# xhchrn/D-LADMM

Hardware: AMD Instinct MI355X
Metric: samples/sec through d=15 D-LADMM forward (m=256,n=512); %HBM-roofline (higher is better)
Workload: dtype f32; 1 GPU; DLADMMNet_scalar (V4) forward m=256 n=512 K=15 B=65536/GPU, all layers' Z/E/L/T written + fused per-layer L1L1 objective; variant=v4, m=256, n=512, layers=15, batch_per_gpu=65536, global_batch=65536, keep_all=True, parallelism=batch-shard dp1 (one RCCL all-reduce of [K,2] sums)

## Files before the change

### d-ladmm_amd/_lib.py

```python
from __future__ import annotations

import ctypes
import os

HERE = os.path.dirname(os.path.abspath(__file__))
LIB_PATH = os.environ.get("DLADMM_LIB") or os.path.join(HERE, "lib", "libdladmm_hip.so")

ABI_VERSION = 6
PREC_F32, PREC_BF16, PREC_F32_SPLIT = 0, 1, 2
MAX_LAYERS = 65536
NSCALAR = 8

F_PER_LAYER, F_BF16_WIDE, F_BWD_PER_LAYER, F_BWD_UNFUSED, F_BWD_NO_ZMASK, F_WGRAD_F32 = \
    1, 2, 4, 8, 16, 32
F_NO_ROWSPLIT = 64
F_NO_XSPLIT = 128
F_ROWSPLIT_ROWP = 256
F_P0_SAVE = 512
F_P0_REUSE = 1024
F_ELZ = 2048
F_ELZ_TAIL = 4096
V1_LENA, V2_LTHETA, V3_FULL, V4_SCALAR, V5_TIED, V6_LASSO = 1, 2, 3, 4, 5, 6
V7_SCALAR_V1E = 7
LOSS_NONE, LOSS_L1L1, LOSS_LASSO = 0, 1, 2
P_BETA1, P_BETA2, P_BETA3, P_SS2, P_SS2B, P_THETA_E, P_THETA_Z, P_S1 = range(8)

EXPORTED = ("dladmm_abi_version", "dladmm_fwd_workspace_bytes", "dladmm_fwd_path",
            "dladmm_fwd_f32", "dladmm_bwd_workspace_bytes", "dladmm_bwd_path", "dladmm_bwd_f32",
            "dladmm_safeguard_f32", "dladmm_safeguard_news_f32", "dladmm_colobj_f32", "dladmm_lena_workspace_bytes",
            "dladmm_lena_f32", "dladmm_scale_f32", "dladmm_error_string")
MU_NONE, MU_EMA, MU_GS, MU_RT = 0, 1, 2, 3

_fp = ctypes.c_void_p
_i32 = ctypes.c_int32
_i64 = ctypes.c_int64


class FwdDesc(ctypes.Structure):
    _fields_ = [
        ("abi_version", _i32), ("variant", _i32), ("m", _i32), ("n", _i32),
        ("batch", _i32), ("layers", _i32), ("keep_all", _i32), ("loss_kind", _i32),
        ("X", _fp), ("ld_x", _i64),
        ("A", _fp), ("ld_a", _i64),
        ("Z0", _fp), ("ld_z0", _i64),
        ("E0", _fp), ("ld_e0", _i64),
        ("L0", _fp), ("ld_l0", _i64),
        ("W", ctypes.POINTER(_fp)), ("ld_w", _i64),
        ("scalar_params", _fp),
        ("row_params", _fp), ("row_stride", _i64),
        ("beta1_elem", ctypes.POINTER(_fp)),
        ("beta2_elem", ctypes.POINTER(_fp)),
        ("ld_beta", _i64),
        ("Z", _fp), ("E", _fp), ("L", _fp), ("T", _fp),
        ("ld_out", _i64),
        ("loss_sums", _fp),
        ("workspace", _fp), ("workspace_bytes", ctypes.c_size_t),
        ("ev_kernel_start", _fp), ("ev_kernel_stop", _fp),
        ("col_loss", _fp),
        ("precision", _i32), ("flags", _i32),
        ("P", _fp),
    ]


class BwdDesc(ctypes.Structure):
    _fields_ = [
        ("fwd", FwdDesc),
        ("gZ", ctypes.POINTER(_fp)), ("gE", ctypes.POINTER(_fp)), ("gL", ctypes.POINTER(_fp)),
        ("gT", ctypes.POINTER(_fp)), ("ld_g", _i64),
        ("loss_kind", _i32), ("gw_sum", _i32), ("loss_coef", _fp),
        ("gW", _fp), ("ld_gw", _i64),
        ("g_scalar", _fp), ("g_row", _fp),
        ("g_beta1_elem", ctypes.POINTER(_fp)), ("g_beta2_elem", ctypes.POINTER(_fp)),
        ("workspace", _fp), ("workspace_bytes", ctypes.c_size_t),
    ]


class SafeguardDesc(ctypes.Structure):
    _fields_ = [
        ("abi_version", _i32), ("m", _i32), ("n", _i32), ("batch", _i32), ("ld", _i64),
        ("Zl", _fp), ("El", _fp), ("Ll", _fp), ("Tl", _fp),
        ("Zk", _fp), ("Ek", _fp), ("Lk", _fp), ("Tk", _fp),
        ("Es", _fp), ("Ts", _fp), ("Ep", _fp),
        ("Zo", _fp), ("Eo", _fp), ("Lo", _fp), ("To", _fp),
        ("mu", _fp), ("norm_out", _fp), ("count", _fp),
        ("beta", ctypes.c_float), ("c", ctypes.c_float), ("delta", ctypes.c_double),
        ("updater", _i32), ("mu_param", ctypes.c_float),
    ]


class SafeguardNewsDesc(ctypes.Structure):
    _fields_ = [
        ("abi_version", _i32), ("m", _i32), ("n", _i32), ("batch", _i32), ("ld", _i64),
        ("X", _fp),
        ("Zl", _fp), ("El", _fp), ("Ll", _fp),
        ("Zk", _fp), ("Ek", _fp), ("Lk", _fp),
        ("En", _fp), ("Znn", _fp), ("Pn", _fp), ("Pnn", _fp),
        ("Zo", _fp), ("Eo", _fp), ("Lo", _fp),
        ("mu", _fp), ("norm_out", _fp), ("count", _fp), ("mask", _fp), ("inv_bs", _fp),
        ("delta", ctypes.c_double), ("updater", _i32), ("mu_param", ctypes.c_float),
    ]


class ColObjDesc(ctypes.Structure):
    _fields_ = [
        ("abi_version", _i32), ("m", _i32), ("n", _i32), ("batch", _i32), ("layers", _i32),
        ("fit_kind", _i32),
        ("Z", _fp), ("z_layer_stride", _i64), ("ld_z", _i64),
        ("E", _fp), ("e_layer_stride", _i64), ("ld_e", _i64),
        ("T", _fp), ("t_layer_stride", _i64), ("ld_t", _i64),
        ("Zref", _fp), ("ld_zref", _i64),
        ("Eref", _fp), ("ld_eref", _i64),
        ("reg", _fp), ("fit", _fp), ("dz", _fp), ("de", _fp),
    ]


class LenaDesc(ctypes.Structure):
    _fields_ = [
        ("abi_version", _i32), ("m", _i32), ("n", _i32), ("batch", _i32), ("layers", _i32),
        ("mode", _i32), ("alpha", ctypes.c_float), ("inv_mb", ctypes.c_float),
        ("inv_nb", ctypes.c_float), ("lx_negate", _i32),
        ("X", _fp), ("ld_x", _i64), ("A", _fp), ("ld_a", _i64),
        ("E", _fp), ("L", _fp), ("layer_stride", _i64), ("ld", _i64),
        ("sums", _fp),
        ("gE", _fp), ("gL", _fp), ("g_layer_stride", _i64), ("ld_g", _i64),
        ("coef", _fp),
        ("workspace", _fp), ("workspace_bytes", ctypes.c_size_t),
    ]


_LIB = None


def lib():
    global _LIB
    if _LIB is not None:
        return _LIB
    if not os.path.exists(LIB_PATH):
        raise RuntimeError(
            f"dladmm: HIP library not built ({LIB_PATH} missing); run "
            "`python -c 'import __graft_entry__ as g; g.build()'` or `make -C d-ladmm_amd`")
    import torch
    L = ctypes.CDLL(LIB_PATH)
    L.dladmm_abi_version.restype = ctypes.c_int
    L.dladmm_abi_version.argtypes = []
    L.dladmm_fwd_workspace_bytes.restype = ctypes.c_size_t
    L.dladmm_fwd_workspace_bytes.argtypes = [ctypes.POINTER(FwdDesc)]
    L.dladmm_fwd_path.restype = ctypes.c_int
    L.dladmm_fwd_path.argtypes = [ctypes.POINTER(FwdDesc)]
    L.dladmm_fwd_f32.restype = ctypes.c_int
    L.dladmm_fwd_f32.argtypes = [ctypes.POINTER(FwdDesc), ctypes.c_void_p]
    L.dladmm_bwd_workspace_bytes.restype = ctypes.c_size_t
    L.dladmm_bwd_workspace_bytes.argtypes = [ctypes.POINTER(BwdDesc)]
    L.dladmm_bwd_path.restype = ctypes.c_int
    L.dladmm_bwd_path.argtypes = [ctypes.POINTER(BwdDesc)]
    L.dladmm_bwd_f32.restype = ctypes.c_int
    L.dladmm_bwd_f32.argtypes = [ctypes.POINTER(BwdDesc), ctypes.c_void_p]
    L.dladmm_safeguard_f32.restype = ctypes.c_int
    L.dladmm_safeguard_f32.argtypes = [ctypes.POINTER(SafeguardDesc), ctypes.c_void_p]
    L.dladmm_safeguard_news_f32.restype = ctypes.c_int
    L.dladmm_safeguard_news_f32.argtypes = [ctypes.POINTER(SafeguardNewsDesc), ctypes.c_void_p]
    L.dladmm_colobj_f32.restype = ctypes.c_int
    L.dladmm_colobj_f32.argtypes = [ctypes.POINTER(ColObjDesc), ctypes.c_void_p]
    L.dladmm_lena_workspace_bytes.restype = ctypes.c_size_t
    L.dladmm_lena_workspace_bytes.argtypes = [ctypes.POINTER(LenaDesc)]
    L.dladmm_lena_f32.restype = ctypes.c_int
    L.dladmm_lena_f32.argtypes = [ctypes.POINTER(LenaDesc), ctypes.c_void_p]
    L.dladmm_scale_f32.restype = ctypes.c_int
    L.dladmm_scale_f32.argtypes = [ctypes.c_void_p, ctypes.c_int64, ctypes.c_void_p, ctypes.c_void_p]
    L.dladmm_error_string.restype = ctypes.c_char_p
    L.dladmm_error_string.argtypes = [ctypes.c_int]
    if L.dladmm_abi_version() != ABI_VERSION:
        raise RuntimeError("dladmm: library ABI version mismatch; rebuild")
    _LIB = L
    return L


def check(code: int):
    if code != 0:
        msg = lib().dladmm_error_string(code).decode()
        if code < 0:
            raise ValueError(f"{msg} (code {code})")
        raise RuntimeError(f"dladmm HIP error: {msg} (code {code})")


def ptr_array(ptrs):
    arr = (_fp * max(len(ptrs), 1))()
    for i, p in enumerate(ptrs):
        arr[i] = p
    return arr
```

### d-ladmm_amd/csrc/dladmm_capi.hip

```cpp
#include <math.h>
#include <stdlib.h>

#include <vector>

#include "dladmm_common.h"
#include "dladmm_wgrad_x3.h"
#include "dladmm_internal.h"

namespace dladmm {

constexpr int kPackBatch = 64;

struct PackArgs {
  const float* src[kPackBatch];
  int R, C, RB, CB;
  int order;
  int64_t ld;
  float* dst;
  float sign;
  const float* scal;
  int trans;
  int t0;
  int bf16;
  int vec;
};
static_assert(sizeof(PackArgs) <= 2048, "kernel argument size");

__global__ __launch_bounds__(256) void pack_frags_kernel(const PackArgs p) {
  const int t = blockIdx.y;
  const int64_t fr = (int64_t)blockIdx.x * 4 + (threadIdx.x >> 6);
  if (fr >= (int64_t)p.RB * p.CB) return;
  const int lane = threadIdx.x & 63;
  int ib, jb;
  if (p.order == 0) { ib = (int)(fr / p.CB); jb = (int)(fr % p.CB); }
  else if (p.order == 1) { ib = (int)(fr % p.RB); jb = (int)(fr / p.RB); }
  else { const int64_t q = fr >> 1; jb = (int)(q % p.CB); ib = 2 * (int)(q / p.CB) + (int)(fr & 1); }
  const float f = p.sign * (p.scal ? p.scal[(p.t0 + t) * DLADMM_NSCALAR + DLADMM_P_S1] : 1.0f);
  const int row = 16 * ib + (lane & 15);
  if (p.bf16) {
    const int c8 = 32 * jb + 8 * (lane >> 4);
    const float* s8 = p.src[t];
    bf16x8 v;
    if (p.vec && !p.trans && row < p.R && c8 + 8 <= p.C) {
      const f32x4* q4 = reinterpret_cast<const f32x4*>(s8 + (int64_t)row * p.ld + c8);
      const f32x4 lo = q4[0], hi = q4[1];
#pragma unroll
      for (int q = 0; q < 4; ++q) {
        v[q] = (__bf16)(f * lo[q]);
        v[4 + q] = (__bf16)(f * hi[q]);
      }
      reinterpret_cast<bf16x8*>(p.dst)[((int64_t)t * p.RB * p.CB + fr) * 64 + lane] = v;
      return;
    }
#pragma unroll
    for (int q = 0; q < 8; ++q) {
      const float x = (row < p.R && c8 + q < p.C)
                          ? f * (p.trans ? s8[(int64_t)(c8 + q) * p.ld + row]
                                         : s8[(int64_t)row * p.ld + c8 + q])
                          : 0.0f;
      v[q] = (__bf16)x;
    }
    reinterpret_cast<bf16x8*>(p.dst)[((int64_t)t * p.RB * p.CB + fr) * 64 + lane] = v;
    return;
  }
  const int c0 = 16 * jb + 4 * (lane >> 4);
  const float* s = p.src[t];
  f32x4 v;
  if (p.vec && !p.trans && row < p.R && c0 + 4 <= p.C) {
    const f32x4 x = *reinterpret_cast<const f32x4*>(s + (int64_t)row * p.ld + c0);
#pragma unroll
    for (int q = 0; q < 4; ++q) v[q] = f * x[q];
    reinterpret_cast<f32x4*>(p.dst)[((int64_t)t * p.RB * p.CB + fr) * 64 + lane] = v;
    return;
  }
#pragma unroll
  for (int q = 0; q < 4; ++q)
    v[q] = (row < p.R && c0 + q < p.C)
               ? f * (p.trans ? s[(int64_t)(c0 + q) * p.ld + row] : s[(int64_t)row * p.ld + c0 + q])
               : 0.0f;
  reinterpret_cast<f32x4*>(p.dst)[((int64_t)t * p.RB * p.CB + fr) * 64 + lane] = v;
}

__global__ __launch_bounds__(256) void zero_fill_kernel(uint32_t* p, int64_t words,
                                                        uint8_t* tail, int ntail) {
  const int64_t i0 = (int64_t)blockIdx.x * 256 + threadIdx.x;
  for (int64_t i = i0; i < words; i += (int64_t)gridDim.x * 256) p[i] = 0u;
  if (i0 < ntail) tail[i0] = 0;
}
inline hipError_t zero_async(void* p, size_t bytes, hipStream_t s) {
  if (bytes == 0) return hipSuccess;
  const uintptr_t a = (uintptr_t)p;
  const size_t head = (4 - (a & 3)) & 3;
  if (head) {
    hipLaunchKernelGGL(zero_fill_kernel, dim3(1), dim3(256), 0, s, (uint32_t*)nullptr,
                       (int64_t)0, (uint8_t*)p, (int)(head < bytes ? head : bytes));
    if (hipError_t e = hipGetLastError()) return e;
    if (head >= bytes) return hipSuccess;
    p = (uint8_t*)p + head;
    bytes -= head;
  }
  const int64_t words = (int64_t)(bytes / 4);
  const int ntail = (int)(bytes & 3);
  int64_t blocks = (words + 255) / 256;
  blocks = blocks < 1 ? 1 : (blocks > 1024 ? 1024 : blocks);
  hipLaunchKernelGGL(zero_fill_kernel, dim3((unsigned)blocks), dim3(256), 0, s, (uint32_t*)p,
                     words, (uint8_t*)p + 4 * words, ntail);
  return hipGetLastError();
}

__global__ __launch_bounds__(256) void zero_2d_kernel(float* p, int64_t ld, int cols, int rows) {
  const int64_t t = (int64_t)blockIdx.x * 256 + threadIdx.x;
  if (t < (int64_t)rows * cols) p[(t / cols) * ld + t % cols] = 0.0f;
}
inline hipError_t zero_2d_async(float* p, int64_t ld, int cols, int rows, hipStream_t s) {
  const int64_t total = (int64_t)rows * cols;
  if (total == 0) return hipSuccess;
  hipLaunchKernelGGL(zero_2d_kernel, dim3((unsigned)((total + 255) / 256)), dim3(256), 0, s, p, ld,
                     cols, rows);
  return hipGetLastError();
}

constexpr int kPtrChunk = 64;
struct PtrChunk {
  const void* p[kPtrChunk];
  const void** dst;
  int n;
};
__global__ __launch_bounds__(64) void ptr_table_kernel(const PtrChunk c) {
  if ((int)threadIdx.x < c.n) c.dst[threadIdx.x] = c.p[threadIdx.x];
}
inline hipError_t write_ptr_table(const void* const* src, int n, const void** dst, hipStream_t s) {
  for (int b = 0; b < n; b += kPtrChunk) {
    PtrChunk c{};
    c.n = n - b < kPtrChunk ? n - b : kPtrChunk;
    for (int i = 0; i < c.n; ++i) c.p[i] = src[b + i];
    c.dst = dst + b;
    hipLaunchKernelGGL(ptr_table_kernel, dim3(1), dim3(64), 0, s, c);
    if (hipError_t e = hipGetLastError()) return e;
  }
  return hipSuccess;
}

typedef _Float16 f16x8_t __attribute__((ext_vector_type(8)));
struct X3PackArgs {
  const float* src[kPackBatch];
  int R, C, RB, KS, t0;
  int64_t ld;
  float sign;
  f16x8_t* dst;
  unsigned* umax;
  int* wexp;
};
static_assert(sizeof(X3PackArgs) <= 2048, "kernel argument size");

__global__ __launch_bounds__(256) void absmax_kernel(const X3PackArgs p) {
  const int t = blockIdx.y;
  const float* src = p.src[t];
  const int64_t total = (int64_t)p.R * p.C;
  float mx = 0.0f;
  for (int64_t i = (int64_t)blockIdx.x * 256 + threadIdx.x; i < total; i += (int64_t)gridDim.x * 256)
    mx = fmaxf(mx, fabsf(src[(i / p.C) * p.ld + i % p.C]));
#pragma unroll
  for (int o = 32; o > 0; o >>= 1) mx = fmaxf(mx, __shfl_xor(mx, o, 64));
  __shared__ float red[4];
  if ((threadIdx.x & 63) == 0) red[threadIdx.x >> 6] = mx;
  __syncthreads();
  if (threadIdx.x == 0) {
    mx = fmaxf(fmaxf(red[0], red[1]), fmaxf(red[2], red[3]));
    atomicMax(p.umax + p.t0 + t, __float_as_uint(mx));
  }
}

__global__ __launch_bounds__(256) void pack_x3_kernel(const X3PackArgs p) {
  const int t = blockIdx.y;
  const int st = blockIdx.x * 4 + (threadIdx.x >> 6);
  if (st >= p.RB * p.KS) return;
  const int lane = threadIdx.x & 63;
  const int ib = st / p.KS, ks = st % p.KS;
  int sw = 15 - __builtin_amdgcn_frexp_expf(__uint_as_float(p.umax[p.t0 + t]));
  sw = sw < -126 ? -126 : (sw > 126 ? 126 : sw);
  if (st == 0 && lane == 0) p.wexp[p.t0 + t] = sw;
  const float f = p.sign * __builtin_amdgcn_ldexpf(1.0f, sw);
  const float* src = p.src[t];
  const int row = 16 * ib + (lane & 15);
  f16x8_t hi, lo;
#pragma unroll
  for (int q = 0; q < 8; ++q) {
    const int c = 32 * ks + 16 * (q >> 2) + 4 * (lane >> 4) + (q & 3);
    const float x = (row < p.R && c < p.C) ? src[(int64_t)row * p.ld + c] * f : 0.0f;
    const _Float16 h = (_Float16)x;
    hi[q] = h;
    lo[q] = (_Float16)(x - (float)h);
  }
  f16x8_t* d = p.dst + ((int64_t)t * p.RB * p.KS + st) * 128;
  d[lane] = hi;
  d[64 + lane] = lo;
}

__global__ __launch_bounds__(256) void col_loss_kernel(const float* part, int nslice, int ldl,
                                                       int B, float* out) {
  const int r = blockIdx.y;
  const int b = blockIdx.x * 256 + threadIdx.x;
  if (b >= B) return;
  float s = 0.0f;
  for (int sl = 0; sl < nslice; ++sl) s += part[((int64_t)r * nslice + sl) * ldl + b];
  out[(int64_t)r * B + b] = s;
}

__global__ __launch_bounds__(1024) void param_reduce_kernel(const float* part, int stride,
                                                            int cnt_m, int cnt_n, double* sums) {
  __shared__ double red[1024];
  const int sl = blockIdx.x;
  if (sl == DLADMM_P_S1) {
    if (threadIdx.x == 0) sums[sl] = 0.0;
    return;
  }
  const int cnt = (sl == DLADMM_P_THETA_Z || sl == DLADMM_P_S1) ? cnt_n : cnt_m;
  double s = 0.0;
  for (int w = threadIdx.x; w < cnt; w += 1024) s += (double)part[(int64_t)sl * stride + w];
  red[threadIdx.x] = s;
  __syncthreads();
  for (int o = 512; o > 0; o >>= 1) {
    if ((int)threadIdx.x < o) red[threadIdx.x] += red[threadIdx.x + o];
    __syncthreads();
  }
  if (threadIdx.x == 0) sums[sl] = red[0];
}

__device__ __forceinline__ double fixed_sum_1024(const float* row, int nw, double* red) {
  double acc8[8] = {0, 0, 0, 0, 0, 0, 0, 0};
  int wv = threadIdx.x;
  for (; wv + 7 * 1024 < nw; wv += 8 * 1024) {
#pragma unroll
    for (int u = 0; u < 8; ++u) acc8[u] += (double)row[wv + u * 1024];
  }
  for (int u = 0; wv < nw; wv += 1024, ++u) acc8[u & 7] += (double)row[wv];
  double s = 0.0;
#pragma unroll
  for (int u = 0; u < 8; ++u) s += acc8[u];
  red[threadIdx.x] = s;
  __syncthreads();
  for (int o = 512; o > 0; o >>= 1) {
    if ((int)threadIdx.x < o) red[threadIdx.x] += red[threadIdx.x + o];
    __syncthreads();
  }
  return red[0];
}

__global__ __launch_bounds__(1024) void loss_reduce_kernel(const float* part, int nw, double* sums) {
  __shared__ double red[1024];
  const int i = blockIdx.x;
  const double s = fixed_sum_1024(part + (int64_t)i * nw, nw, red);
  if (threadIdx.x == 0) sums[i] = s;
}

__global__ __launch_bounds__(1024) void row_reduce_kernel(const float* part, int nw, int prs,
                                                          int ors, int m, int n, unsigned mask,
                                                          double* out) {
  __shared__ double red[1024];
  const int i = blockIdx.x;
  const int row = i % ors, ks = i / ors;
  const int slot = ks % 8;
  const bool ok = ((mask >> slot) & 1u) && row < (slot == DLADMM_P_THETA_Z ? n : m);
  if (!ok) {
    if (threadIdx.x == 0) out[i] = 0.0;
    return;
  }
  const double s = fixed_sum_1024(part + ((int64_t)ks * prs + row) * nw, nw, red);
  if (threadIdx.x == 0) out[i] = s;
}

}

namespace dladmm {

inline size_t align256(size_t x) { return (x + 255) & ~(size_t)255; }

inline int pick_shape(int m, int n) {
  for (int i = 0; i < kNumShapes; ++i)
    if (m <= kShapeMP[i] && n <= kShapeNP[i]) return i;
  return -1;
}

inline int ceil_div(int a, int b) { return (a + b - 1) / b; }

struct Plan {
  int path;
  int shape, MP, NP, tiles;
  int KB1, KB2, SB1, SB2, MBp1, MBp2, slices1, slices2, gx;
  int nslots;
  int ldl;
  int nbp;
  bool narrow;
  size_t off_ap, off_wp, off_v, off_zb, off_zw, off_ew, off_lw, off_loss, total;
  size_t off_btab;
  size_t off_xch, off_xcnt;
  size_t off_wexp, off_umax;
  bool p0;
  size_t off_p0;
  int64_t ldzw;
};

inline bool fits_32bit(const dladmm_fwd_desc* d);

inline int validate(const dladmm_fwd_desc* d) {
  if (!d) return DLADMM_E_NULL;
  if (d->abi_version != DLADMM_ABI_VERSION) return DLADMM_E_ABI_VERSION;
  if (d->variant < DLADMM_V1_LENA || d->variant > DLADMM_V7_SCALAR_V1E) return DLADMM_E_VARIANT;
  if (d->m < 1 || d->n < 1 || d->batch < 1) return DLADMM_E_SHAPE;
  if (d->layers < 1 || d->layers > DLADMM_MAX_LAYERS) return DLADMM_E_LAYERS;
  if (d->loss_kind < 0 || d->loss_kind > 2) return DLADMM_E_UNSUPPORTED;
  if (!d->X || !d->A || !d->Z0 || !d->E0 || !d->L0 || !d->W || !d->Z || !d->E || !d->L)
    return DLADMM_E_NULL;
  for (int k = 0; k < d->layers; ++k)
    if (!d->W[k]) return DLADMM_E_NULL;
  if (d->loss_kind && !d->loss_sums) return DLADMM_E_NULL;
  if (d->col_loss && !d->loss_kind) return DLADMM_E_UNSUPPORTED;
  if (d->precision != DLADMM_PREC_F32 && d->precision != DLADMM_PREC_BF16 &&
      d->precision != DLADMM_PREC_F32_SPLIT)
    return DLADMM_E_UNSUPPORTED;
  const int v = d->variant;
  if (v == DLADMM_V2_LTHETA || v == DLADMM_V3_FULL) {
    if (!d->row_params) return DLADMM_E_NULL;
    if (d->row_stride < d->m || d->row_stride < d->n) return DLADMM_E_SHAPE;
  } else if (!d->scalar_params) {
    return DLADMM_E_NULL;
  }
  if (v == DLADMM_V1_LENA) {
    if (!d->beta1_elem || !d->beta2_elem) return DLADMM_E_NULL;
    for (int k = 0; k < d->layers; ++k)
      if (!d->beta1_elem[k] || !d->beta2_elem[k]) return DLADMM_E_NULL;
    if (d->ld_beta < d->batch) return DLADMM_E_SHAPE;
  }
  const int64_t B = d->batch;
  if (d->ld_x < B || d->ld_z0 < B || d->ld_e0 < B || d->ld_l0 < B || d->ld_out < B)
    return DLADMM_E_SHAPE;
  if (d->ld_a < d->n || d->ld_w < d->m) return DLADMM_E_SHAPE;
  const bool elz = (d->flags & DLADMM_F_ELZ) != 0;
  if (v == DLADMM_V7_SCALAR_V1E || elz) {
    if (d->precision != DLADMM_PREC_F32 || (d->flags & DLADMM_F_PER_LAYER) ||
        pick_shape(d->m, d->n) < 0 || !fits_32bit(d))
      return DLADMM_E_UNSUPPORTED;
    if (v == DLADMM_V7_SCALAR_V1E && d->P && !elz) return DLADMM_E_UNSUPPORTED;
  }
  if (elz) {
    if (v != DLADMM_V4_SCALAR && v != DLADMM_V5_TIED && v != DLADMM_V7_SCALAR_V1E)
      return DLADMM_E_UNSUPPORTED;
    if (!d->keep_all || d->loss_kind) return DLADMM_E_UNSUPPORTED;
  }
  if ((d->flags & DLADMM_F_ELZ_TAIL) && (!elz || !d->P)) return DLADMM_E_UNSUPPORTED;
  return 0;
}

inline bool fits_32bit(const dladmm_fwd_desc* d) {
  const int64_t lim = (int64_t)1 << 31;
  const int64_t mx = d->m > d->n ? d->m : d->n;
  return !(mx * d->ld_x * 4 >= lim || mx * d->ld_z0 * 4 >= lim || mx * d->ld_e0 * 4 >= lim ||
           mx * d->ld_l0 * 4 >= lim || mx * d->ld_out * 4 >= lim ||
           (d->variant == DLADMM_V1_LENA && mx * d->ld_beta * 4 >= lim));
}

inline bool x3_layout_ok(const dladmm_fwd_desc* d) {
  auto al = [](const void* p) { return ((uintptr_t)p & 15) == 0; };
  return d->batch % 4 == 0 && d->ld_out % 4 == 0 && d->ld_z0 % 4 == 0 && al(d->Z0) &&
         al(d->Z) && al(d->E) && al(d->L) && (!d->T || al(d->T));
}

inline bool shared_weight(const dladmm_fwd_desc* d) {
  for (int k = 1; k < d->layers; ++k)
    if (d->W[k] != d->W[0]) return false;
  return true;
}

inline bool use_wgrad_x3(bool x3w, const WgradArgs& wa) { return x3w && wgrad_x3_fits(wa); }

inline int device_cus() {
  static const int n = [] {
    int dev = 0, v = 0;
    if (hipGetDevice(&dev) != hipSuccess ||
        hipDeviceGetAttribute(&v, hipDeviceAttributeMultiprocessorCount, dev) != hipSuccess)
      return 256;
    return v > 0 ? v : 256;
  }();
  return n;
}

#ifndef DLADMM_RS_PER_CU
#define DLADMM_RS_PER_CU 3
#endif
inline bool use_rowsplit(const dladmm_fwd_desc* d, int shape) {
  const bool rowv = d->variant == DLADMM_V2_LTHETA || d->variant == DLADMM_V3_FULL;
  return rs_supports(shape, d->variant) && (!rowv || (d->flags & DLADMM_F_ROWSPLIT_ROWP)) &&
         d->precision == DLADMM_PREC_F32 &&
         !(d->flags & DLADMM_F_NO_ROWSPLIT) &&
         ceil_div(d->batch, 16) <= DLADMM_RS_PER_CU * device_cus();
}

inline bool use_xsplit(const dladmm_fwd_desc* d, int shape) {
  return use_rowsplit(d, shape) && !(d->flags & (DLADMM_F_NO_XSPLIT | DLADMM_F_ELZ)) &&
         xs_grid(d->batch) <= device_cus();
}

inline int make_plan(const dladmm_fwd_desc* d, Plan* p) {
  *p = Plan{};
  const int s = pick_shape(d->m, d->n);
  const int K = d->layers;
  const int64_t B = d->batch;
  const bool force_layered = (d->flags & DLADMM_F_PER_LAYER) != 0;
  const bool bf16 = d->precision == DLADMM_PREC_BF16;
  if (s >= 0 && fits_32bit(d) && !force_layered && d->precision == DLADMM_PREC_F32_SPLIT &&
      x3_supports(d->variant) && x3_layout_ok(d)) {
    p->path = 4;
    p->shape = s < 1 ? 1 : s;
    p->MP = kShapeMP[p->shape];
    p->NP = kShapeNP[p->shape];
    p->tiles = ceil_div(d->batch, kTileCols);
    p->ldl = p->tiles * kTileCols;
    p->nslots = p->ldl;
    p->ldzw = p->ldl;
    const size_t tb = (size_t)p->MP * p->NP * 2 * sizeof(_Float16);
    const int nw = shared_weight(d) ? 1 : K;
    p->off_ap = 0;
    p->off_wp = align256(tb);
    p->off_wexp = p->off_wp + align256(tb * nw);
    p->off_umax = p->off_wexp + align256((size_t)(nw + 1) * sizeof(int));
    p->off_zw = p->off_umax + align256((size_t)(nw + 1) * sizeof(unsigned));
    const bool lean = !d->keep_all && K > 1;
    p->off_loss = p->off_zw + (lean ? align256((size_t)2 * d->n * p->ldzw * sizeof(float)) : 0);
    p->off_btab = p->off_loss + align256((size_t)2 * K * p->nslots * sizeof(float));
    p->total = p->off_btab +
               (d->variant == DLADMM_V1_LENA ? align256((size_t)2 * K * sizeof(void*)) : 0);
    return 0;
  }
  if (s >= 0 && fits_32bit(d) && !force_layered && !bf16) {
    p->path = use_xsplit(d, s) ? 6 : use_rowsplit(d, s) ? 5 : 1;
    p->shape = s;
    p->MP = kShapeMP[s];
    p->NP = kShapeNP[s];
    p->tiles = ceil_div(d->batch, kTileCols);
    p->ldl = p->path >= 5 ? ceil_div(d->batch, 16) * 16 : p->tiles * kTileCols;
    p->nslots = p->ldl;
    const size_t frag_bytes = (size_t)p->MP * p->NP * sizeof(float);
    p->off_ap = 0;
    p->off_wp = align256(frag_bytes);
    p->off_loss = p->off_wp + align256(frag_bytes * (shared_weight(d) ? 1 : K));
    p->off_btab = p->off_loss + align256((size_t)2 * K * p->nslots * sizeof(float));
    p->total = p->off_btab +
               (d->variant == DLADMM_V1_LENA ? align256((size_t)2 * K * sizeof(void*)) : 0);
    if (p->path == 1 && (d->flags & (DLADMM_F_P0_SAVE | DLADMM_F_P0_REUSE)) &&
        !(d->flags & DLADMM_F_ELZ) &&
        d->precision == DLADMM_PREC_F32 && p0_supports(s, d->variant) &&
        (int64_t)p->MP * p->ldl * 4 < ((int64_t)1 << 31)) {
      p->p0 = true;
      p->off_p0 = p->total;
      p->total += align256((size_t)p->MP * p->ldl * sizeof(float));
    }
    if (p->path == 6) {
      const size_t groups = (size_t)xs_grid(d->batch) / 4;
      p->off_xch = p->total;
      p->off_xcnt = p->off_xch + align256(groups * xs_group_floats() * sizeof(float));
      p->total = p->off_xcnt + align256(groups * 64 * sizeof(unsigned));
    }
    return 0;
  }
  p->path = bf16 ? 3 : 2;
  const int MB = ceil_div(d->m, 16), NB = ceil_div(d->n, 16);
  p->KB1 = bf16 ? ceil_div(d->m, 32) : MB;
  p->KB2 = bf16 ? ceil_div(d->n, 32) : NB;
  p->SB1 = bf16 ? kTileBlocks : (NB >= 32 ? 32 : 16);
  p->SB2 = bf16 ? kTileBlocks : (MB >= 32 ? 32 : 16);
  p->MBp1 = ceil_div(NB, p->SB1) * p->SB1;
  p->MBp2 = ceil_div(MB, p->SB2) * p->SB2;
  p->slices1 = p->MBp1 / p->SB1;
  p->slices2 = p->MBp2 / p->SB2;
  p->narrow = bf16 && !(d->flags & DLADMM_F_BF16_WIDE);
  const int cols = bf16 ? bf16_tile_cols(p->narrow) : kLayerCols;
  p->gx = ceil_div(d->batch, cols);
  p->ldl = p->gx * cols;
  p->nbp = p->ldl / 16;
  p->nslots = p->ldl * (p->slices1 > p->slices2 ? p->slices1 : p->slices2) * (bf16 ? 2 : 1);
  const size_t fb = (size_t)kFrag * sizeof(float);
  p->off_ap = 0;
  p->off_wp = align256(fb * p->KB2 * p->MBp2);
  p->off_v = p->off_wp + align256(fb * p->KB1 * p->MBp1 * (shared_weight(d) ? 1 : K));
  p->off_zb = p->off_v + align256(bf16 ? fb * p->KB1 * p->nbp : (size_t)d->m * B * sizeof(float));
  p->off_zw = p->off_zb + (bf16 ? align256(fb * p->KB2 * p->nbp) : 0);
  const bool lean = !d->keep_all && K > 1;
  p->off_ew = p->off_zw + (lean ? align256((size_t)d->n * B * sizeof(float)) : 0);
  p->off_lw = p->off_ew + (lean ? align256((size_t)d->m * B * sizeof(float)) : 0);
  p->off_loss = p->off_lw + (lean ? align256((size_t)d->m * B * sizeof(float)) : 0);
  p->total = p->off_loss + align256((size_t)2 * K * p->nslots * sizeof(float));
  return 0;
}

inline hipError_t pack(const float* const* srcs, int T, int R, int C, int64_t ld, int RB, int CB,
                       int order, float* dst, hipStream_t s, float sign = 1.0f,
                       const float* scal = nullptr, int trans = 0, int t0 = 0, int bf16 = 0) {
  for (int b = 0; b < T; b += kPackBatch) {
    const int nb = T - b < kPackBatch ? T - b : kPackBatch;
    PackArgs pa{};
    pa.trans = trans; pa.t0 = t0 + b;
    for (int t = 0; t < nb; ++t) pa.src[t] = srcs[b + t];
    pa.R = R; pa.C = C; pa.RB = RB; pa.CB = CB; pa.order = order; pa.ld = ld;
    pa.dst = dst + (size_t)b * RB * CB * kFrag;
    pa.sign = sign; pa.scal = scal; pa.bf16 = bf16;
    pa.vec = ld % 4 == 0 ? 1 : 0;
    for (int t = 0; t < nb; ++t)
      if ((uintptr_t)pa.src[t] & 15) pa.vec = 0;
    hipLaunchKernelGGL(pack_frags_kernel, dim3((RB * CB + 3) / 4, nb), dim3(256), 0, s, pa);
    if (hipError_t e = hipGetLastError()) return e;
  }
  return hipSuccess;
}

inline unsigned long long* dbg_ptr() {
#if defined(X3_STAMP) && X3_STAMP
  static unsigned long long* const p = [] {
    const char* e = getenv("DLADMM_DBG_PTR");
    return e ? (unsigned long long*)strtoull(e, nullptr, 0) : nullptr;
  }();
  return p;
#else
  return nullptr;
#endif
}

inline int run_fused(const dladmm_fwd_desc* d, const Plan& p, char* ws, hipStream_t s) {
  float* Ap = (float*)(ws + p.off_ap);
  float* Wp = (float*)(ws + p.off_wp);
  float* lossp = (float*)(ws + p.off_loss);
  const int MB = p.MP / 16, NB = p.NP / 16;
  const float* asrc[1] = {d->A};
  const bool shared = shared_weight(d);
  const bool p0_reuse = p.p0 && !(d->flags & DLADMM_F_P0_SAVE);
  if (!p0_reuse)
    if (hipError_t e = pack(asrc, 1, d->m, d->n, d->ld_a, MB, NB, 2, Ap, s)) return (int)e;
  if (hipError_t e = pack(d->W, shared ? 1 : d->layers, d->n, d->m, d->ld_w, NB, MB, 2, Wp, s,
                          -1.0f))
    return (int)e;
  FusedArgs a{};
  a.m = d->m; a.n = d->n; a.B = d->batch; a.K = d->layers;
  a.keep_all = d->keep_all ? 1 : 0; a.loss_kind = d->loss_kind; a.ldl = p.ldl;
  a.elz = (d->flags & DLADMM_F_ELZ) ? ((d->flags & DLADMM_F_ELZ_TAIL) ? 2 : 1) : 0;
  a.X = d->X; a.ldx = d->ld_x;
  a.Z0 = d->Z0; a.ldz0 = d->ld_z0;
  a.E0 = d->E0; a.lde0 = d->ld_e0;
  a.L0 = d->L0; a.ldl0 = d->ld_l0;
  a.Ap = Ap; a.Wp = Wp;
  a.wstep = shared ? 0 : 1;
  a.scal = d->scalar_params;
  a.rowp = d->row_params; a.rstride = d->row_stride;
  a.ldb = d->ld_beta;
  if (d->variant == DLADMM_V1_LENA) {
    const void** tab = (const void**)(ws + p.off_btab);
    if (hipError_t e = write_ptr_table((const void* const*)d->beta1_elem, d->layers, tab, s))
      return (int)e;
    if (hipError_t e = write_ptr_table((const void* const*)d->beta2_elem, d->layers,
                                       tab + d->layers, s))
      return (int)e;
    a.b1t = (const float* const*)tab;
    a.b2t = (const float* const*)(tab + d->layers);
  }
  a.Zo = d->Z; a.Eo = d->E; a.Lo = d->L; a.To = d->T; a.ldo = d->ld_out;
  a.lossp = lossp;
  a.dbg = dbg_ptr();
  const bool savep = d->P != nullptr && d->keep_all;
  a.Po = savep ? d->P : nullptr;
  if (p.p0) {
    a.P0 = (const float*)(ws + p.off_p0);
    a.ldp0 = p.ldl;
    if (!p0_reuse)
      if (hipError_t e = launch_p0_producer(p.shape, Ap, d->Z0, d->ld_z0, d->n, d->batch,
                                            (float*)(ws + p.off_p0), p.ldl, p.tiles, s))
        return (int)e;
  }
  if (d->ev_kernel_start) {
    if (hipError_t e = hipEventRecord((hipEvent_t)d->ev_kernel_start, s)) return (int)e;
  }
  if (p.path == 6) {
    a.xch = (float*)(ws + p.off_xch);
    a.xstride = (int64_t)xs_group_floats();
    a.xcnt = (unsigned*)(ws + p.off_xcnt);
    if (hipError_t e = zero_async(a.xcnt, p.total - p.off_xcnt, s)) return (int)e;
  }
  hipError_t e = p.path == 6 ? launch_fused_xs(p.shape, d->variant, a, s)
                 : p.path == 5
                    ? launch_fused_rs(p.shape, d->variant, a, ceil_div(d->batch, 16), s)
                 : a.elz ? launch_fused_shape_elz(p.shape, d->variant, a, p.tiles, s)
                 : p0_reuse
                    ? (savep ? launch_fused_shape_p0_savep : launch_fused_shape_p0)(
                          p.shape, d->variant, a, p.tiles, s)
                    : (savep ? launch_fused_shape_savep : launch_fused_shape)(p.shape, d->variant,
                                                                             a, p.tiles, s);
  if (e) return (int)e;
  if (d->ev_kernel_stop) {
    if (hipError_t e = hipEventRecord((hipEvent_t)d->ev_kernel_stop, s)) return (int)e;
  }
  return 0;
}

inline hipError_t pack_x3(const float* const* srcs, int T, int R, int C, int64_t ld, int RB,
                          int KS, float sign, _Float16* dst, unsigned* umax, int* wexp, int t0,
                          hipStream_t s) {
  for (int b = 0; b < T; b += kPackBatch) {
    const int nb = T - b < kPackBatch ? T - b : kPackBatch;
    X3PackArgs pa{};
    for (int t = 0; t < nb; ++t) pa.src[t] = srcs[b + t];
    pa.R = R; pa.C = C; pa.RB = RB; pa.KS = KS; pa.t0 = t0 + b; pa.ld = ld; pa.sign = sign;
    pa.dst = reinterpret_cast<f16x8_t*>(dst) + (size_t)b * RB * KS * 128;
    pa.umax = umax; pa.wexp = wexp;
    const int blocks = ceil_div((int)(((int64_t)R * C + 255) / 256), 8);
    hipLaunchKernelGGL(absmax_kernel, dim3(blocks < 64 ? blocks : 64, nb), dim3(256), 0, s, pa);
    if (hipError_t e = hipGetLastError()) return e;
    hipLaunchKernelGGL(pack_x3_kernel, dim3(ceil_div(RB * KS, 4), nb), dim3(256), 0, s, pa);
    if (hipError_t e = hipGetLastError()) return e;
  }
  return hipSuccess;
}

inline int run_fused_x3(const dladmm_fwd_desc* d, const Plan& p, char* ws, hipStream_t s) {
  _Float16* Ap = (_Float16*)(ws + p.off_ap);
  _Float16* Wp = (_Float16*)(ws + p.off_wp);
  int* wexp = (int*)(ws + p.off_wexp);
  unsigned* umax = (unsigned*)(ws + p.off_umax);
  const int MB = p.MP / 16, NB = p.NP / 16, KS1 = p.MP / 32, KS2 = p.NP / 32;
  const bool shared = shared_weight(d);
  const int nw = shared ? 1 : d->layers;
  if (hipError_t e = zero_async(umax, (size_t)(nw + 1) * sizeof(unsigned), s)) return (int)e;
  const float* asrc[1] = {d->A};
  if (hipError_t e = pack_x3(asrc, 1, d->m, d->n, d->ld_a, MB, KS2, 1.0f, Ap, umax, wexp, 0, s))
    return (int)e;
  if (hipError_t e = pack_x3(d->W, nw, d->n, d->m, d->ld_w, NB, KS1, -1.0f, Wp, umax, wexp, 1, s))
    return (int)e;
  FusedArgs a{};
  a.m = d->m; a.n = d->n; a.B = d->batch; a.K = d->layers;
  a.keep_all = d->keep_all ? 1 : 0; a.loss_kind = d->loss_kind; a.ldl = p.ldl;
  a.X = d->X; a.ldx = d->ld_x;
  a.Z0 = d->Z0; a.ldz0 = d->ld_z0;
  a.E0 = d->E0; a.lde0 = d->ld_e0;
  a.L0 = d->L0; a.ldl0 = d->ld_l0;
  a.Ap = (const float*)Ap; a.Wp = (const float*)Wp;
  a.wstep = shared ? 0 : 1;
  a.scal = d->scalar_params;
  a.Zo = d->Z; a.Eo = d->E; a.Lo = d->L; a.To = d->T; a.ldo = d->ld_out;
  a.lossp = (float*)(ws + p.off_loss);
  a.wexp = wexp;
  a.Zw = (float*)(ws + p.off_zw); a.ldzw = p.ldzw;
  a.dbg = dbg_ptr();
  if (d->variant == DLADMM_V1_LENA) {
    a.ldb = d->ld_beta;
    const void** tab = (const void**)(ws + p.off_btab);
    if (hipError_t e = write_ptr_table((const void* const*)d->beta1_elem, d->layers, tab, s))
      return (int)e;
    if (hipError_t e = write_ptr_table((const void* const*)d->beta2_elem, d->layers,
                                       tab + d->layers, s))
      return (int)e;
    a.b1t = (const float* const*)tab;
    a.b2t = (const float* const*)(tab + d->layers);
  }
  if (d->ev_kernel_start) {
    if (hipError_t e = hipEventRecord((hipEvent_t)d->ev_kernel_start, s)) return (int)e;
  }
  const bool savep = d->P != nullptr && d->keep_all;
  a.Po = savep ? d->P : nullptr;
  if (hipError_t e = (savep ? launch_fused_x3_shape_savep : launch_fused_x3_shape)(
          p.shape, d->variant, a, p.tiles, s))
    return (int)e;
  if (d->ev_kernel_stop) {
    if (hipError_t e = hipEventRecord((hipEvent_t)d->ev_kernel_stop, s)) return (int)e;
  }
  return 0;
}

inline int run_layered(const dladmm_fwd_desc* d, const Plan& p, char* ws, hipStream_t s) {
  const int K = d->layers, m = d->m, n = d->n;
  const int64_t B = d->batch;
  float* Ap = (float*)(ws + p.off_ap);
  float* Wp = (float*)(ws + p.off_wp);
  float* V = (float*)(ws + p.off_v);
  float* Zw = (float*)(ws + p.off_zw);
  float* Ew = (float*)(ws + p.off_ew);
  float* Lw = (float*)(ws + p.off_lw);
  float* lossp = (float*)(ws + p.off_loss);
  const size_t wl = (size_t)kFrag * p.KB1 * p.MBp1;
  const int bf = p.path == 3 ? 1 : 0;
  const int sb1 = p.SB1, sb2 = p.SB2;
  char* Vb = ws + p.off_v;
  char* Zb = ws + p.off_zb;
  auto launch = [&](int phase, const LayerArgs& la, dim3 grid, int sb) -> hipError_t {
    return bf ? launch_tile_bf16(phase, d->variant, p.narrow, la, grid, s)
              : launch_layer(phase, d->variant, la, grid, sb, s);
  };
  const float* asrc[1] = {d->A};
  if (hipError_t e = pack(asrc, 1, m, n, d->ld_a, p.MBp2, p.KB2, 1, Ap, s, 1.0f, nullptr, 0, 0, bf))
    return (int)e;
  const bool shared = shared_weight(d);
  if (hipError_t e = pack(d->W, shared ? 1 : K, n, m, d->ld_w, p.MBp1, p.KB1, 1, Wp, s, 1.0f,
                          nullptr, 0, 0, bf))
    return (int)e;
  if (d->loss_kind) {
    if (hipError_t e = zero_async(lossp, (size_t)2 * K * p.nslots * sizeof(float), s))
      return (int)e;
  }
  const bool lean = !d->keep_all;
  const int64_t ldo = d->ld_out;
  const int64_t zl = (int64_t)n * ldo, ml = (int64_t)m * ldo;
  LayerArgs a{};
  a.m = m; a.n = n; a.B = d->batch; a.K = K;
  a.loss_kind = d->loss_kind; a.nslots = p.nslots; a.ldl = p.ldl;
  a.X = d->X; a.ldx = d->ld_x;
  a.Vo = bf ? nullptr : V; a.ldv = B;
  a.nbp = p.nbp;
  a.scal = d->scalar_params;
  a.rowp = d->row_params; a.rstride = d->row_stride;
  a.ldb = d->ld_beta;
  a.lossp = d->loss_kind ? lossp : nullptr;
  const dim3 g1(p.gx, p.slices1), g2(p.gx, p.slices2);
  const bool v1 = d->variant == DLADMM_V1_LENA;
  auto run = [&](int phase, const LayerArgs& la, dim3 grid, int sb) -> hipError_t {
    return launch(phase, la, grid, sb);
  };
  if (d->ev_kernel_start) {
    if (hipError_t e = hipEventRecord((hipEvent_t)d->ev_kernel_start, s)) return (int)e;
  }
  {
    LayerArgs b = a;
    b.k = -1; b.KB = p.KB2; b.MBp = p.MBp2; b.Krows = n; b.Wp = Ap;
    b.S = d->Z0; b.ldS = d->ld_z0;
    if (bf) {
      if (hipError_t e = pack_state_bf16(d->Z0, d->ld_z0, n, B, p.KB2, p.nbp, Zb, s))
        return (int)e;
      b.S = (const float*)Zb;
      b.Pb = Vb; b.pb_kb = p.KB1;
    }
    b.Eprev = d->E0; b.ldep = d->ld_e0; b.Lprev = d->L0; b.ldlp = d->ld_l0;
    b.ldo = ldo;
    b.To = (d->T && !lean) ? d->T : nullptr;
    b.b1n_e = v1 ? d->beta1_elem[0] : nullptr;
    if (hipError_t e = run(2, b, g2, sb2)) return (int)e;
  }
  for (int k = 0; k < K; ++k) {
    const bool last = k == K - 1;
    const float* Zp = k == 0 ? d->Z0 : (lean ? Zw : d->Z + (k - 1) * zl);
    const int64_t ldzp = k == 0 ? d->ld_z0 : (lean ? B : ldo);
    const float* Ep = k == 0 ? d->E0 : (lean ? Ew : d->E + (k - 1) * ml);
    const int64_t ldep = k == 0 ? d->ld_e0 : (lean ? B : ldo);
    const float* Lp = k == 0 ? d->L0 : (lean ? Lw : d->L + (k - 1) * ml);
    const int64_t ldlp = k == 0 ? d->ld_l0 : (lean ? B : ldo);
    float* Zo = lean ? (last ? d->Z : Zw) : d->Z + k * zl;
    float* Eo = lean ? (last ? d->E : Ew) : d->E + k * ml;
    float* Lo = lean ? (last ? d->L : Lw) : d->L + k * ml;
    const int64_t ldout = (lean && !last) ? B : ldo;
    LayerArgs b = a;
    b.k = k; b.KB = p.KB1; b.MBp = p.MBp1; b.Krows = m; b.Wp = Wp + (shared ? 0 : k * wl);
    b.S = bf ? (const float*)Vb : V; b.ldS = B;
    b.Zprev = Zp; b.ldzp = ldzp;
    b.Zo = Zo; b.ldo = ldout;
    if (bf) { b.Pb = Zb; b.pb_kb = p.KB2; }
    if (hipError_t e = run(0, b, g1, sb1)) return (int)e;
    LayerArgs c = a;
    c.k = k; c.KB = p.KB2; c.MBp = p.MBp2; c.Krows = n; c.Wp = Ap;
    c.S = bf ? (const float*)Zb : Zo; c.ldS = ldout;
    if (bf && !last) { c.Pb = Vb; c.pb_kb = p.KB1; }
    c.Eprev = Ep; c.ldep = ldep; c.Lprev = Lp; c.ldlp = ldlp;
    c.Eo = Eo; c.Lo = Lo; c.ldo = ldout;
    c.To = d->T ? (lean ? (last ? d->T : nullptr) : d->T + (k + 1) * ml) : nullptr;
    if (v1) {
      c.b1e = d->beta1_elem[k];
      c.b2e = d->beta2_elem[k];
      c.b1n_e = k + 1 < K ? d->beta1_elem[k + 1] : nullptr;
    }
    if (hipError_t e = run(1, c, g2, sb2)) return (int)e;
  }
  if (d->ev_kernel_stop) {
    if (hipError_t e = hipEventRecord((hipEvent_t)d->ev_kernel_stop, s)) return (int)e;
  }
  return 0;
}

struct BwdPlan {
  Plan fwd;
  int MB, NB, SBm, MBpm, NBpn, slices_m, slices_n, gx;
  int64_t Bpad, Rn, Rm;
  int nslots, ncg;
  int wtiles, nchunks; int64_t chunk;
  int wgl;
  bool saved_p;
  bool x3w;
  size_t off_a1, off_at, off_m, off_mt, off_az, off_ae, off_al, off_at_, off_gp, off_var,
      off_part, off_part2, off_wpart, off_s1dot, total;
  bool rev;
  int rtiles, rncg;
  int rnrow;
  bool rrs;
  bool rxs;
  size_t off_rxcnt, off_rxch;
  int64_t Rn2, Rm2;
  size_t off_ratp, off_rmtp, off_gu, off_rvar, off_rpart, off_rptab, off_rrow;
};

inline bool bwd_flag(const dladmm_fwd_desc& f, int flag) { return (f.flags & flag) != 0; }

inline int validate_bwd(const dladmm_bwd_desc* d) {
  if (!d) return DLADMM_E_NULL;
  if (int e = validate(&d->fwd)) return e;
  const dladmm_fwd_desc& f = d->fwd;
  if (!f.keep_all || !f.T) return DLADMM_E_UNSUPPORTED;
  if (f.variant == DLADMM_V7_SCALAR_V1E || (f.flags & (DLADMM_F_ELZ | DLADMM_F_ELZ_TAIL)))
    return DLADMM_E_UNSUPPORTED;
  if (f.precision != DLADMM_PREC_F32 && f.precision != DLADMM_PREC_F32_SPLIT)
    return DLADMM_E_UNSUPPORTED;
  if (!fits_32bit(&f)) return DLADMM_E_UNSUPPORTED;
  {
    const int64_t mx = f.m > f.n ? f.m : f.n, lim = (int64_t)1 << 31;
    const int64_t bpad = (f.batch + 15) / 16 * 16;
    if (mx * bpad * 4 >= lim || mx * d->ld_g * 4 >= lim) return DLADMM_E_UNSUPPORTED;
  }
  if (!d->gW) return DLADMM_E_NULL;
  if (d->ld_gw < f.m) return DLADMM_E_SHAPE;
  if ((d->gZ || d->gE || d->gL || d->gT) && d->ld_g < f.batch) return DLADMM_E_SHAPE;
  if (d->loss_kind < 0 || d->loss_kind > 2) return DLADMM_E_UNSUPPORTED;
  if (d->loss_kind && !d->loss_coef) return DLADMM_E_NULL;
  const int v = f.variant;
  if (v >= DLADMM_V4_SCALAR && !d->g_scalar) return DLADMM_E_NULL;
  if ((v == DLADMM_V2_LTHETA || v == DLADMM_V3_FULL) && !d->g_row) return DLADMM_E_NULL;
  if (v == DLADMM_V1_LENA) {
    if (!d->g_beta1_elem || !d->g_beta2_elem) return DLADMM_E_NULL;
    for (int k = 0; k < f.layers; ++k)
      if (!d->g_beta1_elem[k] || !d->g_beta2_elem[k]) return DLADMM_E_NULL;
  }
  return 0;
}

inline int64_t round_up(int64_t x, int64_t q) { return (x + q - 1) / q * q; }
inline int64_t K_of(const dladmm_fwd_desc& f) { return f.layers; }

inline size_t rev_ws_cap() {
  static size_t cache[64] = {0};
  int dev = 0;
  if (hipGetDevice(&dev) != hipSuccess || dev < 0 || dev >= 64) return (size_t)64 << 30;
  if (!cache[dev]) {
    size_t total = 0;
    cache[dev] = hipDeviceTotalMem(&total, dev) == hipSuccess && total ? total / 4
                                                                        : (size_t)64 << 30;
  }
  return cache[dev];
}

inline int make_bwd_plan(const dladmm_bwd_desc* d, BwdPlan* p) {
  *p = BwdPlan{};
  const dladmm_fwd_desc& f = d->fwd;
  dladmm_fwd_desc f32 = f;
  f32.precision = DLADMM_PREC_F32;
  if (int e = make_plan(&f32, &p->fwd)) return e;
  p->x3w = f.precision == DLADMM_PREC_F32_SPLIT && !bwd_flag(f, DLADMM_F_WGRAD_F32);
  p->saved_p = f.P != nullptr && f.keep_all &&
               (p->fwd.path == 1 || p->fwd.path == 4 || p->fwd.path >= 5);
  const int m = f.m, n = f.n;
  const int64_t B = f.batch;
  p->MB = ceil_div(m, 16);
  p->NB = ceil_div(n, 16);
  p->SBm = 16;
  p->MBpm = ceil_div(p->MB, p->SBm) * p->SBm;
  p->NBpn = ceil_div(p->NB, 32) * 32;
  p->slices_m = p->MBpm / p->SBm;
  p->slices_n = p->NBpn / 16;
  p->gx = ceil_div(f.batch, kBwdCols);
  p->Bpad = round_up(B, 16);
  p->Rn = round_up(n, 128);
  p->Rm = round_up(m, 128);
  p->ncg = p->gx * kBwdWaves;
  p->nslots = p->ncg * (p->slices_m > p->slices_n ? p->slices_m : p->slices_n);
  const int64_t rs = f.row_stride > 0 ? f.row_stride : 1;
  const int64_t part_floats = 8 * (p->nslots > rs * p->ncg ? (int64_t)p->nslots : rs * p->ncg);
  p->rev = false;
  const bool cot_ok = !(d->gZ || d->gE || d->gL || d->gT) || d->ld_g == f.ld_out;
  const bool v1_ok = f.variant != DLADMM_V1_LENA || f.ld_beta == f.ld_out;
  if (p->saved_p && reverse_supports(f.variant) && cot_ok && v1_ok &&
      f.ld_e0 == f.ld_out && f.ld_l0 == f.ld_out && !bwd_flag(f, DLADMM_F_BWD_PER_LAYER)) {
    const int MP = kShapeMP[p->fwd.shape], NP = kShapeNP[p->fwd.shape];
    const int64_t bpad = p->x3w ? round_up(B, 32) : p->Bpad;
    p->Rn2 = round_up(NP, 128);
    p->Rm2 = round_up(MP, 128);
    const int64_t lim = (int64_t)1 << 31;
    const bool rowv = f.variant == DLADMM_V2_LTHETA || f.variant == DLADMM_V3_FULL;
    const size_t rev_bytes = (size_t)(K_of(f) + 1) * MP * NP * 4 +
                             (size_t)K_of(f) * (p->Rn2 + p->Rm2 + MP) * bpad * 4 +
                             (rowv ? (size_t)8 * K_of(f) * (MP > NP ? MP : NP) *
                                         ((B + 63) / 64 * 4) * 4 : 0);
    if ((int64_t)NP * bpad * 4 < lim && 2 * (p->Rm2 + MP) * bpad * 4 < lim &&
        rev_bytes <= rev_ws_cap()) {
      p->rev = true;
      p->Bpad = bpad;
      p->Rn = p->Rn2;
      p->Rm = p->Rm2;
      p->rrs = p->fwd.path >= 5 && f.precision == DLADMM_PREC_F32 &&
               reverse_rs_supports(p->fwd.shape, f.variant) &&
               ceil_div((int)f.batch, 16) <= device_cus();
      p->rxs = p->rrs && p->fwd.path == 6;
      p->rtiles = p->rxs ? xs_grid(f.batch)
                  : p->rrs ? ceil_div(f.batch, 16) : ceil_div(f.batch, kTileCols);
      p->rncg = p->rtiles * kWaves;
      p->rnrow = p->rrs ? ceil_div((int)f.batch, 16) : p->rncg;
    }
  }
  p->wtiles = (int)((p->Rn / 128) * (p->Rm / 128));
  const int q = p->x3w && p->rev ? 32 : 16;
  const int64_t steps = p->Bpad / q;
  int64_t nch = (512 + p->wtiles - 1) / p->wtiles;
  if (nch > steps) nch = steps;
  if (nch < 1) nch = 1;
  p->chunk = ceil_div((int)steps, (int)nch) * q;
  p->nchunks = (int)((p->Bpad + p->chunk - 1) / p->chunk);
  const size_t fb = (size_t)kFrag * sizeof(float);
  const size_t colb = (size_t)p->Bpad * sizeof(float);
  size_t o = 0;
  if (p->rev) {
    const size_t wb = (size_t)kShapeMP[p->fwd.shape] * kShapeNP[p->fwd.shape] * sizeof(float);
    const size_t K = (size_t)f.layers;
    p->off_ratp = o; o += align256(wb);
    p->off_rmtp = o; o += align256(wb * K);
    p->off_gu = o; o += align256(colb * p->Rn2 * K);
    p->off_rvar = o; o += align256(colb * (p->Rm2 + kShapeMP[p->fwd.shape]) * K);
    p->off_rpart = o; o += align256(sizeof(float) * DLADMM_NSCALAR * K * p->rncg);
    p->off_rxcnt = o;
    if (p->rxs) o += align256(sizeof(unsigned) * 64 * (size_t)(p->rtiles / 4));
    const size_t lpart = sizeof(float) * (size_t)p->nchunks * n * m;
    p->wgl = (int)((size_t)256 * 1024 * 1024 / lpart);
    if (p->wgl < 1) p->wgl = 1;
    if (p->wgl > (int)K) p->wgl = (int)K;
    p->off_wpart = o; o += align256(lpart * p->wgl);
    p->off_s1dot = o; o += align256(sizeof(double) * (size_t)s1_dot_blocks(n, m) * K);
    p->off_rptab = o; o += align256(sizeof(void*) * (size_t)(RT_NTAB * K + 1));
    const bool rowk = f.variant == DLADMM_V2_LTHETA || f.variant == DLADMM_V3_FULL;
    p->off_rrow = o;
    const int RS = kShapeMP[p->fwd.shape] > kShapeNP[p->fwd.shape] ? kShapeMP[p->fwd.shape]
                                                                    : kShapeNP[p->fwd.shape];
    if (rowk) o += align256(sizeof(float) * 8 * K * (size_t)RS * p->rnrow);
    p->off_rxch = o;
    if (p->rxs) o += align256(sizeof(float) * rev_xs_group_floats() * (size_t)(p->rtiles / 4));
    p->total = o;
    return 0;
  }
  p->off_a1 = o; o += align256(fb * p->NB * p->MBpm);
  p->off_at = o; o += align256(fb * p->MB * p->NBpn);
  p->off_m = o; o += align256(fb * p->MB * p->NBpn);
  p->off_mt = o; o += align256(fb * p->NB * p->MBpm);
  p->off_az = o; o += align256(colb * p->Rn);
  p->off_ae = o; o += align256(colb * m);
  p->off_al = o; o += align256(colb * m);
  p->off_at_ = o; o += align256(colb * m);
  p->off_gp = o; o += align256(colb * m);
  p->off_var = o; o += align256(colb * p->Rm);
  p->off_part = o; o += align256(sizeof(float) * part_floats);
  p->off_part2 = o; o += align256(sizeof(float) * part_floats);
  p->off_wpart = o; o += align256(sizeof(float) * (size_t)p->nchunks * n * m);
  p->off_s1dot = o; o += align256(sizeof(double) * (size_t)s1_dot_blocks(n, m));
  p->total = o;
  return 0;
}

inline int run_reverse(const dladmm_bwd_desc* d, const BwdPlan& p, char* ws, hipStream_t s) {
  const dladmm_fwd_desc& f = d->fwd;
  const int K = f.layers, m = f.m, n = f.n;
  const int shape = p.fwd.shape, MP = kShapeMP[shape], NP = kShapeNP[shape];
  const int MB = MP / 16, NB = NP / 16;
  float* Atp = (float*)(ws + p.off_ratp);
  float* Mtp = (float*)(ws + p.off_rmtp);
  float* GU = (float*)(ws + p.off_gu);
  float* VAR = (float*)(ws + p.off_rvar);
  float* rpart = (float*)(ws + p.off_rpart);
  float* wpart = (float*)(ws + p.off_wpart);
  const int64_t ldw = p.Bpad, gus = p.Rn2 * ldw, vas = (p.Rm2 + MP) * ldw;
  const float* asrc[1] = {f.A};
  if (hipError_t e = pack(asrc, 1, n, m, f.ld_a, NB, MB, 2, Atp, s, 1.0f, nullptr, 1))
    return (int)e;
  if (hipError_t e = pack(f.W, K, m, n, f.ld_w, MB, NB, 2, Mtp, s, -1.0f, f.scalar_params, 1, 0))
    return (int)e;
  if (hipError_t e = zero_async(rpart, p.off_wpart - p.off_rpart, s)) return (int)e;
  for (int k = 0; k < K && (p.Rn2 > NP || p.Rm2 > MP); ++k) {
    if (p.Rn2 > NP)
      if (hipError_t e = zero_async(GU + k * gus + NP * ldw,
                                        (size_t)(p.Rn2 - NP) * ldw * sizeof(float), s))
        return (int)e;
    if (p.Rm2 > MP)
      if (hipError_t e = zero_async(VAR + k * vas + MP * ldw,
                                        (size_t)(p.Rm2 - MP) * ldw * sizeof(float), s))
        return (int)e;
  }
  RevArgs r{};
  r.m = m; r.n = n; r.B = (int)f.batch; r.K = K;
  r.loss_kind = d->loss_kind; r.ncg = p.rncg;
  if (f.variant == DLADMM_V2_LTHETA || f.variant == DLADMM_V3_FULL) r.ncg = p.rnrow;
  r.Bw = p.Bpad;
  r.X = f.X; r.ldx = f.ld_x;
  r.E0 = f.E0; r.lde0 = f.ld_e0;
  r.L0 = f.L0; r.ldl0 = f.ld_l0;
  r.Z = f.Z; r.E = f.E; r.L = f.L; r.T = f.T; r.P = f.P; r.ldo = f.ld_out;
  r.Atp = Atp; r.Mtp = Mtp;
  r.scal = f.scalar_params;
  r.lcoef = d->loss_kind ? d->loss_coef : nullptr;
  r.GU = GU; r.VAR = VAR; r.ldw = ldw; r.gus = gus; r.vas = vas;
  r.aer = p.Rm2;
  r.part = rpart;
  {
    std::vector<const void*> tab((size_t)RT_NTAB * K + 1, nullptr);
    auto put = [&](int t, const void* const* src, int cnt) {
      for (int k = 0; src && k < cnt; ++k) tab[rev_tab_at(t, K, k)] = src[k];
    };
    put(RT_GZ, (const void* const*)d->gZ, K);
    put(RT_GE, (const void* const*)d->gE, K);
    put(RT_GL, (const void* const*)d->gL, K);
    put(RT_GT, (const void* const*)d->gT, K + 1);
    if (f.variant == DLADMM_V1_LENA) {
      put(RT_B1, (const void* const*)f.beta1_elem, K);
      put(RT_B2, (const void* const*)f.beta2_elem, K);
      put(RT_GB1, (const void* const*)d->g_beta1_elem, K);
      put(RT_GB2, (const void* const*)d->g_beta2_elem, K);
    }
    const void** ptab = (const void**)(ws + p.off_rptab);
    if (hipError_t e = write_ptr_table(tab.data(), (int)tab.size(), ptab, s)) return (int)e;
    r.ptab = (const float* const*)ptab;
  }
  r.has_gz = d->gZ ? 1 : 0;
  r.has_cot = (d->gE || d->gL || d->gT) ? 1 : 0;
  const bool rowk = f.variant == DLADMM_V2_LTHETA || f.variant == DLADMM_V3_FULL;
  if (rowk) {
    r.rowp = f.row_params; r.rstride = f.row_stride;
    r.rpart = (float*)(ws + p.off_rrow);
  }
  if (p.rxs) {
    r.xch = (float*)(ws + p.off_rxch);
    r.xstride = (int64_t)rev_xs_group_floats();
    r.xcnt = (unsigned*)(ws + p.off_rxcnt);
  }
  if (hipError_t e = p.rxs ? launch_reverse_xs(shape, f.variant, r, s)
                     : p.rrs ? launch_reverse_rs(shape, f.variant, r, p.rtiles, s)
                             : launch_reverse_shape(shape, f.variant, r, p.rtiles, s))
    return (int)e;
  const bool tied = d->gw_sum != 0, v5 = f.variant == DLADMM_V5_TIED;
  double* s1dot = (double*)(ws + p.off_s1dot);
  const int nbd = s1_dot_blocks(n, m);
  if (tied)
    if (hipError_t e = zero_2d_async(d->gW, d->ld_gw, m, n, s)) return (int)e;
  bool wsame = true;
  for (int k = 1; k < K; ++k) wsame = wsame && f.W[k] == f.W[0];
  const int wgl = v5 && !wsame ? 1 : p.wgl;
  for (int khi = K - 1; khi >= 0; khi -= wgl) {
    const int nl = khi + 1 < wgl ? khi + 1 : wgl, klo = khi - nl + 1;
    WgradArgs wa{};
    wa.G = GU + klo * gus; wa.V = VAR + klo * vas; wa.ld = ldw; wa.n = n; wa.m = m;
    wa.NBp16 = (int)(p.Rn2 / 16); wa.MBp16 = (int)(p.Rm2 / 16);
    wa.Bpad = p.Bpad; wa.chunk = p.chunk; wa.nchunks = p.nchunks; wa.part = wpart;
    wa.gls = gus; wa.vls = vas; wa.pls = (int64_t)p.nchunks * n * m;
    if (hipError_t e = (use_wgrad_x3(p.x3w, wa) ? launch_wgrad_x3 : launch_wgrad)(wa, p.wtiles, s, nl))
      return (int)e;
    WredArgs ra{};
    ra.part = wpart; ra.pls = wa.pls; ra.nchunks = p.nchunks; ra.nm = (int64_t)n * m;
    ra.scal = f.scalar_params; ra.klo = klo; ra.nl = nl; ra.tied = tied ? 1 : 0;
    ra.gW = d->gW; ra.gls = (int64_t)n * d->ld_gw; ra.ldgw = d->ld_gw; ra.m = m;
    ra.Wd = v5 ? f.W[klo] : nullptr; ra.ldwd = f.ld_w;
    ra.dotp = v5 ? s1dot : nullptr; ra.nbd = nbd;
    if (hipError_t e = launch_wgrad_reduce_layers(ra, s)) return (int)e;
  }
  if (rowk) {
    unsigned mask = (1u << DLADMM_P_THETA_Z) | (1u << DLADMM_P_BETA1) | (1u << DLADMM_P_BETA3) |
                    (1u << DLADMM_P_BETA2) | (1u << DLADMM_P_THETA_E);
    if (f.variant == DLADMM_V3_FULL) mask |= 1u << DLADMM_P_SS2;
    hipLaunchKernelGGL(row_reduce_kernel, dim3((unsigned)(8 * K * f.row_stride)), dim3(1024), 0,
                       s, (const float*)r.rpart, p.rnrow, MP > NP ? MP : NP, (int)f.row_stride, m,
                       n, mask, d->g_row);
    if (hipError_t e = hipGetLastError()) return (int)e;
  } else if (f.variant != DLADMM_V1_LENA) {
    hipLaunchKernelGGL(loss_reduce_kernel, dim3((unsigned)(DLADMM_NSCALAR * K)), dim3(1024), 0,
                       s, (const float*)rpart, p.rncg, d->g_scalar);
    if (hipError_t e = hipGetLastError()) return (int)e;
  }
  for (int k = 0; k < K && v5; ++k)
    if (hipError_t e = launch_s1_dot_finish(s1dot + (int64_t)k * nbd, n, m,
                                            d->g_scalar + (int64_t)k * DLADMM_NSCALAR +
                                                DLADMM_P_S1, s))
      return (int)e;
  return 0;
}

inline int run_bwd(const dladmm_bwd_desc* d, const BwdPlan& p, char* ws, hipStream_t s) {
  if (p.rev) return run_reverse(d, p, ws, s);
  const dladmm_fwd_desc& f = d->fwd;
  const int K = f.layers, m = f.m, n = f.n;
  const int64_t B = f.batch, ldo = f.ld_out, ldw = p.Bpad;
  const int v = f.variant;
  const bool has_s1 = v >= DLADMM_V4_SCALAR;
  const bool tied = d->gw_sum != 0;
  const bool rowk = v == DLADMM_V2_LTHETA || v == DLADMM_V3_FULL;
  float* A1 = (float*)(ws + p.off_a1);
  float* At = (float*)(ws + p.off_at);
  float* Mp = (float*)(ws + p.off_m);
  float* Mt = (float*)(ws + p.off_mt);
  float* AZ = (float*)(ws + p.off_az);
  float* AE = (float*)(ws + p.off_ae);
  float* AL = (float*)(ws + p.off_al);
  float* AT = (float*)(ws + p.off_at_);
  float* GP = (float*)(ws + p.off_gp);
  float* VAR = (float*)(ws + p.off_var);
  float* const part = (float*)(ws + p.off_part);
  float* wpart = (float*)(ws + p.off_wpart);
  if (hipError_t e = zero_async(ws + p.off_az, p.off_part - p.off_az, s)) return (int)e;
  if (tied) {
    if (hipError_t e = zero_2d_async(d->gW, d->ld_gw, m, n, s)) return (int)e;
  }
  const bool v5 = v == DLADMM_V5_TIED;
  double* s1dot = (double*)(ws + p.off_s1dot);
  const float* asrc[1] = {f.A};
  if (hipError_t e = pack(asrc, 1, m, n, f.ld_a, p.MBpm, p.NB, 1, A1, s)) return (int)e;
  if (hipError_t e = pack(asrc, 1, n, m, f.ld_a, p.NBpn, p.MB, 1, At, s, 1.0f, nullptr, 1))
    return (int)e;
  const int64_t zl = (int64_t)n * ldo, ml = (int64_t)m * ldo;
  BwdArgs a{};
  a.m = m; a.n = n; a.B = (int)B; a.K = K;
  a.nslots = p.nslots; a.ncg = p.ncg;
  a.X = f.X; a.ldx = f.ld_x;
  a.ldg = d->ld_g;
  a.loss_kind = d->loss_kind;
  a.lcoef = d->loss_coef;
  a.AZ = AZ; a.AE = AE; a.AL = AL; a.AT = AT; a.GP = GP; a.VAR = VAR; a.ldw = ldw;
  a.scal = f.scalar_params;
  a.rowp = f.row_params; a.rstride = f.row_stride;
  a.ldb = f.ld_beta;
  a.part = part;
  const dim3 gm(p.gx, p.slices_m), gn(p.gx, p.slices_n);
  const size_t part_bytes = p.off_part2 - p.off_part;
  const bool fuse = p.saved_p && !bwd_flag(f, DLADMM_F_BWD_UNFUSED);
  float* part2 = (float*)(ws + p.off_part2);
  auto partk = [&](int k) { return (fuse && (k & 1)) ? part2 : part; };
  const dim3 gm4(ceil_div((int)B, 64 * kBwdWaves), p.slices_m);
  auto layer_args = [&](BwdArgs& x, int k) {
    x.k = k;
    x.Ep = k ? f.E + (k - 1) * ml : f.E0; x.ldep = k ? ldo : f.ld_e0;
    x.Lp = k ? f.L + (k - 1) * ml : f.L0; x.ldlp = k ? ldo : f.ld_l0;
    x.Zp = k ? f.Z + (k - 1) * zl : f.Z0; x.ldzp = k ? ldo : f.ld_z0;
    x.Tk = f.T + k * ml; x.ldt = ldo;
    x.gZ = d->gZ ? d->gZ[k] : nullptr;
    x.gE = d->gE ? d->gE[k] : nullptr;
    x.gL = d->gL ? d->gL[k] : nullptr;
    x.gT = d->gT ? d->gT[k + 1] : nullptr;
    if (v == DLADMM_V1_LENA) {
      x.b1e = f.beta1_elem[k]; x.b2e = f.beta2_elem[k];
      x.gb1e = d->g_beta1_elem[k]; x.gb2e = d->g_beta2_elem[k];
    }
    x.part = partk(k);
  };
  if (fuse) {
    if (hipError_t e = zero_async(rowk ? partk(K - 1) : part,
                                      rowk ? part_bytes : 2 * part_bytes, s))
      return (int)e;
    BwdArgs b1 = a;
    layer_args(b1, K - 1);
    b1.Pk = f.P + (int64_t)(K - 1) * ml;
    if (hipError_t e = launch_bwd(4, v, b1, gm4, p.SBm, s)) return (int)e;
  }
  for (int k = K - 1; k >= 0; --k) {
    const float* wsrc[1] = {f.W[k]};
    if (hipError_t e = pack(wsrc, 1, n, m, f.ld_w, p.NBpn, p.MB, 1, Mp, s)) return (int)e;
    if (hipError_t e = pack(wsrc, 1, m, n, f.ld_w, p.MBpm, p.NB, 1, Mt, s, -1.0f,
                            has_s1 ? f.scalar_params : nullptr, 1, k))
      return (int)e;
    if (!fuse && (rowk || k == K - 1))
      if (hipError_t e = zero_async(part, part_bytes, s)) return (int)e;
    layer_args(a, k);
    if (!fuse) {
      BwdArgs b1 = a;
      b1.KB = p.NB; b1.MBp = p.MBpm; b1.Krows = n; b1.Wp = A1;
      b1.S = f.Z + k * zl; b1.ldS = ldo;
      b1.Pk = p.saved_p ? f.P + k * ml : nullptr;
      if (hipError_t e = launch_bwd(p.saved_p ? 4 : 1, v, b1, p.saved_p ? gm4 : gm, p.SBm, s))
        return (int)e;
    }
    BwdArgs b2 = a;
    b2.KB = p.MB; b2.MBp = p.NBpn; b2.Krows = m;
    b2.Wp = At; b2.S = GP; b2.ldS = ldw;
    b2.Wp2 = Mp; b2.S2 = VAR; b2.ldS2 = ldw;
    b2.Zk = f.Z + k * zl; b2.ldzk = ldo;
    const bool zm = v == DLADMM_V1_LENA || v == DLADMM_V4_SCALAR || v == DLADMM_V5_TIED ||
                    v == DLADMM_V6_LASSO;
    const bool zrow = (v == DLADMM_V2_LTHETA || v == DLADMM_V3_FULL) && !bwd_flag(f, DLADMM_F_BWD_NO_ZMASK);
    b2.zk_mask = (zm || zrow) ? 2 : 0;
    if (zm || zrow) {
      if (hipError_t e = launch_bwd(5, v, b2, dim3(p.gx, p.slices_n / 2), 32, s)) return (int)e;
    }
    if (hipError_t e = launch_bwd(2, v, b2, gn, 16, s)) return (int)e;
    WgradArgs wa{};
    wa.G = AZ; wa.V = VAR; wa.ld = ldw; wa.n = n; wa.m = m;
    wa.NBp16 = (int)(p.Rn / 16); wa.MBp16 = (int)(p.Rm / 16);
    wa.Bpad = p.Bpad; wa.chunk = p.chunk; wa.nchunks = p.nchunks; wa.part = wpart;
    if (hipError_t e = (use_wgrad_x3(p.x3w, wa) ? launch_wgrad_x3 : launch_wgrad)(wa, p.wtiles, s, 1))
      return (int)e;
    float* gWk = tied ? d->gW : d->gW + (int64_t)k * n * d->ld_gw;
    if (hipError_t e = launch_wgrad_reduce(wpart, p.nchunks, n, m,
                                           has_s1 ? f.scalar_params : nullptr, k, tied ? 1 : 0,
                                           gWk, d->ld_gw, s, v5 ? f.W[k] : nullptr, f.ld_w,
                                           v5 ? s1dot : nullptr))
      return (int)e;
    BwdArgs b3 = a;
    b3.KB = p.NB; b3.MBp = p.MBpm; b3.Krows = n; b3.Wp = Mt;
    b3.S = AZ; b3.ldS = ldw;
    if (fuse && k > 0) {
      layer_args(b3, k - 1);
      b3.Pk = f.P + (int64_t)(k - 1) * ml;
      b3.k3 = k;
      b3.Tk3 = f.T + k * ml;
      if (v == DLADMM_V1_LENA) { b3.b1e3 = f.beta1_elem[k]; b3.gb1e3 = d->g_beta1_elem[k]; }
      b3.part3 = partk(k);
      if (rowk)
        if (hipError_t e = zero_async(partk(k - 1), part_bytes, s)) return (int)e;
      if (hipError_t e = launch_bwd(6, v, b3, gm, p.SBm, s)) return (int)e;
    } else {
      if (hipError_t e = launch_bwd(3, v, b3, gm, p.SBm, s)) return (int)e;
    }
    float* const pk = partk(k);
    if (v >= DLADMM_V4_SCALAR) {
      hipLaunchKernelGGL(param_reduce_kernel, dim3(DLADMM_NSCALAR), dim3(1024), 0, s,
                         (const float*)pk, p.nslots, p.gx * kBwdWaves * p.slices_m,
                         p.gx * kBwdWaves * p.slices_n,
                         d->g_scalar + (int64_t)k * DLADMM_NSCALAR);
      if (hipError_t e = hipGetLastError()) return (int)e;
      if (v5)
        if (hipError_t e = launch_s1_dot_finish(s1dot, n, m, d->g_scalar +
                                                (int64_t)k * DLADMM_NSCALAR + DLADMM_P_S1, s))
          return (int)e;
    } else if (rowk) {
      hipLaunchKernelGGL(loss_reduce_kernel, dim3((unsigned)(DLADMM_NSCALAR * f.row_stride)),
                         dim3(1024), 0, s, (const float*)pk, p.ncg,
                         d->g_row + (int64_t)k * DLADMM_NSCALAR * f.row_stride);
      if (hipError_t e = hipGetLastError()) return (int)e;
    }
  }
  return 0;
}

__global__ __launch_bounds__(256) void scale_if_kernel(float* x, int64_t n, const float* s) {
  const float v = *s;
  if (v == 1.0f) return;
  for (int64_t i = (int64_t)blockIdx.x * 256 + threadIdx.x; i < n; i += (int64_t)gridDim.x * 256)
    x[i] *= v;
}

struct LenaPlan {
  int shape, MP, NP, tiles, ldl;
  bool rs;
  size_t off_ap, off_atp, off_part, total;
};

inline int lena_plan(const dladmm_lena_desc* d, LenaPlan* p) {
  *p = LenaPlan{};
  if (!d) return DLADMM_E_NULL;
  if (d->abi_version != DLADMM_ABI_VERSION) return DLADMM_E_ABI_VERSION;
  if (d->m < 1 || d->n < 1 || d->batch < 1) return DLADMM_E_SHAPE;
  if (d->layers < 1 || d->layers > 65535) return DLADMM_E_LAYERS;
  if (d->mode < 0 || d->mode > 2) return DLADMM_E_UNSUPPORTED;
  if (d->lx_negate != 0 && d->lx_negate != 1) return DLADMM_E_UNSUPPORTED;
  if (!d->X || !d->A || !d->E || !d->L) return DLADMM_E_NULL;
  if (d->mode != 1 && !d->sums) return DLADMM_E_NULL;
  if (d->mode != 0 && (!d->gE || !d->gL || !d->coef)) return DLADMM_E_NULL;
  const int64_t B = d->batch;
  if (d->ld < B || d->ld_x < B || d->ld_a < d->n) return DLADMM_E_SHAPE;
  if (d->layers > 1 && d->layer_stride < (int64_t)d->m * d->ld) return DLADMM_E_SHAPE;
  if (d->mode != 0) {
    if (d->ld_g < B) return DLADMM_E_SHAPE;
    if (d->layers > 1 && d->g_layer_stride < (int64_t)d->m * d->ld_g) return DLADMM_E_SHAPE;
  }
  const int s = pick_shape(d->m, d->n);
  if (s < 0) return DLADMM_E_UNSUPPORTED;
  const int64_t lim = (int64_t)1 << 31;
  const int64_t MPs = kShapeMP[s];
  if (MPs * d->ld * 4 >= lim || MPs * d->ld_x * 4 >= lim ||
      (d->mode != 0 && MPs * d->ld_g * 4 >= lim))
    return DLADMM_E_UNSUPPORTED;
  p->shape = s;
  p->MP = kShapeMP[s];
  p->NP = kShapeNP[s];
  p->rs = s == 2 && ceil_div(d->batch, 16) <= device_cus();
  p->tiles = p->rs ? ceil_div(d->batch, 16) : ceil_div(d->batch, kTileCols);
  p->ldl = p->tiles * (p->rs ? 16 : kTileCols);
  if (d->mode != 1 && (int64_t)16 * d->layers * p->ldl >= lim) return DLADMM_E_UNSUPPORTED;
  const size_t fb = (size_t)p->MP * p->NP * sizeof(float);
  p->off_ap = 0;
  p->off_atp = align256(fb);
  p->off_part = p->off_atp + align256(fb);
  p->total = p->off_part +
             (d->mode != 1 ? align256((size_t)4 * d->layers * p->ldl * sizeof(float)) : 0);
  return 0;
}

}

extern "C" {

size_t dladmm_lena_workspace_bytes(const dladmm_lena_desc* d) {
  using namespace dladmm;
  LenaPlan p;
  return lena_plan(d, &p) ? 0 : p.total;
}

int dladmm_lena_f32(const dladmm_lena_desc* d, void* stream) {
  using namespace dladmm;
  LenaPlan p;
  if (int e = lena_plan(d, &p)) return e;
  if (!d->workspace || d->workspace_bytes < p.total) return DLADMM_E_WORKSPACE;
  if (((uintptr_t)d->workspace) & 255) return DLADMM_E_ALIGN;
  hipStream_t s = (hipStream_t)stream;
  char* ws = (char*)d->workspace;
  float* Ap = (float*)(ws + p.off_ap);
  float* Atp = (float*)(ws + p.off_atp);
  const int MB = p.MP / 16, NB = p.NP / 16;
  const float* asrc[1] = {d->A};
  if (hipError_t e = pack(asrc, 1, d->m, d->n, d->ld_a, MB, NB, 2, Ap, s)) return (int)e;
  if (hipError_t e = pack(asrc, 1, d->n, d->m, d->ld_a, NB, MB, 2, Atp, s, 1.0f, nullptr, 1))
    return (int)e;
  LenaArgs a{};
  a.m = d->m; a.n = d->n; a.B = d->batch; a.K = d->layers; a.mode = d->mode; a.ldl = p.ldl;
  a.alpha = d->alpha; a.inv_mb = d->inv_mb; a.inv_nb = d->inv_nb;
  a.xsign = d->lx_negate ? -1.0f : 1.0f;
  for (int i = 0; i < 2; ++i) {
    const double c = i == 0 ? (double)d->alpha : 1.0;
    a.gc[4 * i + 0] = (float)c;
    a.gc[4 * i + 1] = (float)(1.0 + exp(-2.0 * c));
    a.gc[4 * i + 2] = (float)exp(-c);
    a.gc[4 * i + 3] = (float)(exp(c) + exp(-c));
  }
  a.X = d->X; a.ldx = d->ld_x;
  a.E = d->E; a.L = d->L; a.ls = d->layer_stride; a.ld = d->ld;
  a.Ap = Ap; a.Atp = Atp;
  a.part = (float*)(ws + p.off_part);
  a.gE = d->gE; a.gL = d->gL; a.gls = d->g_layer_stride; a.ldg = d->ld_g;
  a.coef = d->coef;
  if (hipError_t e = p.rs ? launch_lena_rs(a, p.tiles, s) : launch_lena(p.shape, a, p.tiles, s))
    return (int)e;
  if (d->mode != 1) {
    hipLaunchKernelGGL(loss_reduce_kernel, dim3((unsigned)(4 * d->layers)), dim3(1024), 0, s,
                       (const float*)a.part, p.ldl, d->sums);
    if (hipError_t e = hipGetLastError()) return (int)e;
  }
  return 0;
}

int dladmm_scale_f32(float* x, int64_t n, const float* s, void* stream) {
  using namespace dladmm;
  if (n < 0) return DLADMM_E_SHAPE;
  if (n == 0) return 0;
  if (!x || !s) return DLADMM_E_NULL;
  int64_t blocks = (n + 255) / 256;
  blocks = blocks > 4096 ? 4096 : blocks;
  hipLaunchKernelGGL(scale_if_kernel, dim3((unsigned)blocks), dim3(256), 0, (hipStream_t)stream,
                     x, n, s);
  return (int)hipGetLastError();
}

int dladmm_abi_version(void) { return DLADMM_ABI_VERSION; }

size_t dladmm_fwd_workspace_bytes(const dladmm_fwd_desc* d) {
  using namespace dladmm;
  if (validate(d)) return 0;
  Plan p;
  if (make_plan(d, &p)) return 0;
  return p.total;
}

int dladmm_fwd_path(const dladmm_fwd_desc* d) {
  using namespace dladmm;
  if (int e = validate(d)) return e;
  Plan p;
  if (int e = make_plan(d, &p)) return e;
  return p.path;
}

int dladmm_fwd_f32(const dladmm_fwd_desc* d, void* stream) {
  using namespace dladmm;
  if (int e = validate(d)) return e;
  Plan p;
  if (int e = make_plan(d, &p)) return e;
  if (!d->workspace || d->workspace_bytes < p.total) return DLADMM_E_WORKSPACE;
  if (((uintptr_t)d->workspace) & 255) return DLADMM_E_ALIGN;
  hipStream_t s = (hipStream_t)stream;
  char* ws = (char*)d->workspace;
  const int rc = p.path == 1 || p.path >= 5 ? run_fused(d, p, ws, s)
                 : p.path == 4 ? run_fused_x3(d, p, ws, s)
                               : run_layered(d, p, ws, s);
  if (rc) return rc;
  if (d->loss_kind) {
    hipLaunchKernelGGL(loss_reduce_kernel, dim3(2 * d->layers), dim3(1024), 0, s,
                       (const float*)(ws + p.off_loss), p.nslots, d->loss_sums);
    if (hipError_t e = hipGetLastError()) return (int)e;
    if (d->col_loss) {
      hipLaunchKernelGGL(col_loss_kernel, dim3(ceil_div(d->batch, 256), 2 * d->layers),
                         dim3(256), 0, s, (const float*)(ws + p.off_loss), p.nslots / p.ldl,
                         p.ldl, d->batch, d->col_loss);
      if (hipError_t e = hipGetLastError()) return (int)e;
    }
  }
  return 0;
}

size_t dladmm_bwd_workspace_bytes(const dladmm_bwd_desc* d) {
  using namespace dladmm;
  if (validate_bwd(d)) return 0;
  BwdPlan p;
  if (make_bwd_plan(d, &p)) return 0;
  return p.total;
}

int dladmm_bwd_path(const dladmm_bwd_desc* d) {
  using namespace dladmm;
  if (int e = validate_bwd(d)) return e;
  BwdPlan p;
  if (int e = make_bwd_plan(d, &p)) return e;
  return p.rev ? (p.rxs ? 3 : p.rrs ? 2 : 1) : 0;
}

int dladmm_bwd_f32(const dladmm_bwd_desc* d, void* stream) {
  using namespace dladmm;
  if (int e = validate_bwd(d)) return e;
  BwdPlan p;
  if (int e = make_bwd_plan(d, &p)) return e;
  if (!d->workspace || d->workspace_bytes < p.total) return DLADMM_E_WORKSPACE;
  if (((uintptr_t)d->workspace) & 255) return DLADMM_E_ALIGN;
  return run_bwd(d, p, (char*)d->workspace, (hipStream_t)stream);
}

const char* dladmm_error_string(int code) {
  switch (code) {
    case 0: return "success";
    case DLADMM_E_ABI_VERSION: return "dladmm: descriptor abi_version mismatch";
    case DLADMM_E_VARIANT: return "dladmm: unknown variant";
    case DLADMM_E_SHAPE: return "dladmm: invalid shape or leading dimension";
    case DLADMM_E_LAYERS: return "dladmm: layers must be in [1, DLADMM_MAX_LAYERS]";
    case DLADMM_E_NULL: return "dladmm: required pointer is NULL";
    case DLADMM_E_WORKSPACE: return "dladmm: workspace missing or too small";
    case DLADMM_E_UNSUPPORTED: return "dladmm: unsupported configuration";
    case DLADMM_E_ALIGN: return "dladmm: workspace must be 256-byte aligned";
  }
  if (code > 0) return hipGetErrorString((hipError_t)code);
  return "dladmm: unknown error";
}

}
```

### d-ladmm_amd/model.py

```python
from __future__ import annotations

from collections import OrderedDict
from typing import List, Optional

import numpy as np
import torch
import torch.nn as nn

from . import _lib
from .ops import (ForwardResult, PrologueCache, dladmm_backward, dladmm_forward, dladmm_lena,
                  dladmm_scale_)


def _dev(t: torch.Tensor) -> torch.Tensor:
    return t.cuda() if torch.cuda.is_available() else t


class _DLADMMBase(nn.Module):
    VARIANT = 0
    RETURNS_T = False
    WSCALE = 1.0
    NAME = "DLADMMNet"

    def __init__(self, m, n, d, batch_size, A, Z0, E0, L0, layers, *, batch_shard=None):
        super().__init__()
        self.m = m
        self.n = n
        self.d = d
        self.batch_size = batch_size
        self.layers = layers
        self.batch_shard = None
        cols = None
        if batch_shard is not None:
            from .dist import shard_columns
            rank, world = (int(x) for x in batch_shard)
            cols = shard_columns(batch_size, rank, world)
            Z0, E0, L0 = (_shard_cols(t, batch_size, cols, nm)
                          for t, nm in ((Z0, "Z0"), (E0, "E0"), (L0, "L0")))
        self.A = _dev(A)
        self.Z0 = _dev(Z0)
        self.E0 = _dev(E0)
        self.L0 = _dev(L0)
        self._pcols = batch_size if cols is None else cols[1] - cols[0]
        self._register_params()
        self._init_fc()
        if cols is not None:
            self.batch_shard = (cols[0], cols[1], batch_size)
            self.world = (rank, world)
        self.to(self.A.device)

    def _plist(self, name, shape, value):
        pl = nn.ParameterList()
        for _ in range(self.layers):
            pl.append(nn.Parameter(value * torch.ones(*shape, dtype=torch.float32)))
        setattr(self, name, pl)

    def _register_params(self):
        raise NotImplementedError

    def _init_fc(self):
        for mod in self.modules():
            if isinstance(mod, nn.Linear):
                w = self.A.t() + (1e-3) * torch.randn_like(self.A.t())
                if self.WSCALE != 1.0:
                    w = w * self.WSCALE
                mod.weight = nn.Parameter(w.contiguous())

    def name(self):
        return self.NAME

    def _elem_param_lists(self) -> list:
        return []

    def shard_batch_(self, rank: int, world: int):
        from .dist import shard_columns
        if self.batch_shard is not None:
            raise RuntimeError("dladmm: the module is already a batch shard")
        B = self.Z0.shape[1]
        for pl in self._elem_param_lists():
            if any(q.shape[1] != B for q in pl):
                raise ValueError("dladmm: per-sample parameters and Z0 disagree on the batch")
        c0, c1 = shard_columns(B, rank, world)
        self.Z0 = self.Z0[:, c0:c1].contiguous()
        self.E0 = self.E0[:, c0:c1].contiguous()
        self.L0 = self.L0[:, c0:c1].contiguous()
        for pl in self._elem_param_lists():
            for i in range(len(pl)):
                pl[i] = nn.Parameter(pl[i].detach()[:, c0:c1].contiguous(),
                                     requires_grad=pl[i].requires_grad)
        self._pcols = c1 - c0
        self.batch_shard = (c0, c1, B)
        self.world = (rank, world)
        return self

    def load_state_dict(self, state_dict, strict: bool = True, assign: bool = False):
        if self.batch_shard is not None:
            c0, c1, B = self.batch_shard
            names = {f"{nm}.{k}" for nm in self._elem_names() for k in range(self.layers)}
            sd = OrderedDict(state_dict)
            for key in names & set(sd):
                v = sd[key]
                if torch.is_tensor(v) and v.dim() == 2 and v.shape[1] == B and c1 - c0 != B:
                    sd[key] = v[:, c0:c1]
            state_dict = sd
        return super().load_state_dict(state_dict, strict=strict, assign=assign)

    def _elem_names(self) -> list:
        return [nm for nm, mod in self.named_children() if any(mod is pl for pl in
                                                               self._elem_param_lists())]

    def _weights(self) -> List[torch.Tensor]:
        return [self.fc[k].weight for k in range(self.layers)]

    def _table_spec(self) -> dict:
        raise NotImplementedError

    def _elem_betas(self, cols=None) -> dict:
        return {}

    def _tables(self, dev, cols=None) -> dict:
        out = {}
        for kind, spec in self._table_spec().items():
            R = 1 if kind == "scalar" else max(self.m, self.d)
            rows = {nm: (1 if kind == "scalar" else (self.d if nm == "thz" else self.m))
                    for nm in spec}
            out[f"{kind}_params"] = _assemble_table(self.layers, R, dev, spec, rows)
        out.update(self._elem_betas(cols))
        return out

    def _needs_grad(self) -> bool:
        return torch.is_grad_enabled() and any(p.requires_grad for p in self.parameters())

    precision = "f32"

    reuse_prologue = True

    def _p0_cache(self):
        if not self.reuse_prologue:
            return None
        c = self.__dict__.get("_p0c")
        if c is None:
            c = self.__dict__["_p0c"] = PrologueCache()
        return c

    def invalidate_cache(self):
        c = self.__dict__.get("_p0c")
        if c is not None:
            c.invalidate()

    def run(self, x: torch.Tensor, keep_all: bool = True, loss_kind: int = 0,
            kernel_events=None, want_col_loss: bool = False):
        with torch.no_grad():
            dev = self.A.device
            return dladmm_forward(
                self.VARIANT, x, self.A, [w.detach() for w in self._weights()],
                self.Z0, self.E0, self.L0, keep_all=keep_all, want_T=self.RETURNS_T,
                loss_kind=loss_kind, kernel_events=kernel_events, want_col_loss=want_col_loss,
                precision=self.precision, p0_cache=self._p0_cache(), **self._tables(dev))

    def _forward_layers(self, x, nl: int):
        if self._needs_grad():
            if x.requires_grad:
                raise RuntimeError("dladmm: gradients w.r.t. the input X are not supported (the "
                                   "reference trains the parameters only)")
            if self.precision not in ("f32", "f32_split"):
                raise RuntimeError(f"dladmm: precision {self.precision!r} is inference-only "
                                   "(training runs f32 or f32_split)")
            outs = _DLADMMFunction.apply(self, x, nl, *self.parameters())
            return (list(outs[:nl]), list(outs[nl:2 * nl]), list(outs[2 * nl:3 * nl]),
                    list(outs[3 * nl:]))
        with torch.no_grad():
            tables = _slice_tables(self._tables(self.A.device), nl)
            r = dladmm_forward(self.VARIANT, x, self.A, [w.detach() for w in self._weights()[:nl]],
                               self.Z0, self.E0, self.L0, keep_all=True, want_T=self.RETURNS_T,
                               precision=self.precision, p0_cache=self._p0_cache(), **tables)
        T = [r.T[j] for j in range(nl + 1)] if r.T is not None else None
        return ([r.Z[k] for k in range(nl)], [r.E[k] for k in range(nl)],
                [r.L[k] for k in range(nl)], T)

    def forward(self, x):
        Z, E, L, T = self._forward_layers(x, self.layers)
        if self.RETURNS_T:
            return Z, E, L, T
        return Z, E, L

    def layer_objectives(self, x, alpha: float, kind: str = "l1l1", kernel_events=None,
                         want_col_loss: bool = False):
        lk = {"l1l1": _lib.LOSS_L1L1, "lasso": _lib.LOSS_LASSO}[kind]
        r = self.run(x, loss_kind=lk, kernel_events=kernel_events, want_col_loss=want_col_loss)
        obj = (alpha * r.loss_sums[:, 0] + r.loss_sums[:, 1]) / x.shape[1]
        return r, obj

    def training_loss(self, x, alpha: float, coeffs=None, kind: str = "l1l1",
                      batch: Optional[int] = None, cols=None, lx_sign: float = 1.0,
                      save_cotangents: bool = True):
        K = self.layers
        coeffs = [1.0] * K if coeffs is None else [float(c) for c in coeffs]
        if len(coeffs) != K:
            raise ValueError(f"dladmm: coeffs must have {K} entries")
        if kind not in ("l1l1", "lasso", "lena"):
            raise ValueError(f"dladmm: unknown loss kind {kind!r}")
        if cols is not None and self.batch_shard is not None:
            raise ValueError("dladmm: cols= slices a replicated model; a batch shard "
                             "(shard_batch_) takes its own columns' x directly")
        if batch is None and self.batch_shard is not None:
            batch = self.batch_shard[2]
        if cols is not None:
            cols = (int(cols[0]), int(cols[1]))
            if not (0 <= cols[0] <= cols[1] <= self.Z0.shape[1]) or \
                    x.shape[1] != cols[1] - cols[0]:
                raise ValueError(f"dladmm: cols {cols} do not match x {tuple(x.shape)} and the "
                                 f"model's batch of {self.Z0.shape[1]} columns")
        denom = float(batch if batch is not None else x.shape[1])
        if kind == "lena":
            lx_sign = float(lx_sign)
            if lx_sign not in (1.0, -1.0):
                raise ValueError(f"dladmm: lx_sign must be +1 or -1 (got {lx_sign})")
            if self._needs_grad():
                if x.requires_grad:
                    raise RuntimeError("dladmm: gradients w.r.t. the input X are not supported")
                return _DLADMMLenaLossFunction.apply(self, x, coeffs, float(alpha), denom, cols,
                                                     lx_sign, bool(save_cotangents),
                                                     *self.parameters())
            with torch.no_grad():
                r = self._run_shard(x, cols, loss_kind=_lib.LOSS_L1L1, want_T=False)
                sums = dladmm_lena(x, self.A, r.E, r.L, float(alpha), denom, lx_sign=lx_sign)
                per_layer = _lena_per_layer(r.loss_sums, sums, float(alpha), self.A.shape,
                                            denom, lx_sign)
                c = _coef_tensor(coeffs, per_layer.device)
                return (c * per_layer).sum().to(torch.float32), per_layer.to(torch.float32)
        if self._needs_grad():
            if x.requires_grad:
                raise RuntimeError("dladmm: gradients w.r.t. the input X are not supported")
            return _DLADMMLossFunction.apply(self, x, coeffs, float(alpha), kind, denom, cols,
                                             *self.parameters())
        lk = {"l1l1": _lib.LOSS_L1L1, "lasso": _lib.LOSS_LASSO}[kind]
        with torch.no_grad():
            r = self._run_shard(x, cols, loss_kind=lk, want_T=self.RETURNS_T)
        per_layer = (alpha * r.loss_sums[:, 0] + r.loss_sums[:, 1]) / denom
        c = _coef_tensor(coeffs, per_layer.device)
        return (c * per_layer).sum().to(torch.float32), per_layer.to(torch.float32)

    def _init_state(self, cols=None):
        if cols is None:
            return self.Z0, self.E0, self.L0
        c0, c1 = cols
        return self.Z0[:, c0:c1], self.E0[:, c0:c1], self.L0[:, c0:c1]

    def _run_shard(self, x, cols, **kw):
        dev = self.A.device
        Z0, E0, L0 = self._init_state(cols)
        W = [w.detach() for w in self._weights()]
        kw.setdefault("precision", self.precision)
        kw.setdefault("p0_cache", self._p0_cache())
        return dladmm_forward(self.VARIANT, x, self.A, W, Z0, E0, L0, keep_all=True,
                              **kw, **self._tables(dev, cols))

    GRAD_SLOTS: dict = {}
    PARAM_STEPS = {"beta1": "z", "beta2": "e", "beta3": "l", "ss2": "e", "ss2_1": "e",
                   "ss2_2": "e", "ss1": "z", "active_para": "z", "active_para1": "e"}

    def _fc_key(self, k: int) -> str:
        return "fc.weight" if self._shared_weight() else f"fc.{k}.weight"

    def _param_grads(self, res, nl: int, reach: Optional[dict] = None, cols=None) -> dict:
        out = {}
        rz = reach["z"] if reach else [True] * nl
        kinds = {kind for kind, _ in self.GRAD_SLOTS.values()}
        gs32 = res.g_scalar.to(torch.float32) if "scalar" in kinds else None
        gr32 = res.g_row.to(torch.float32) if "row" in kinds else None
        for name, (kind, slots) in self.GRAD_SLOTS.items():
            steps = self.PARAM_STEPS[name]
            for k in range(nl):
                if reach is not None and not any(reach[s][k] for s in steps):
                    continue
                key = f"{name}.{k}"
                if kind == "scalar":
                    g = (gs32[k, slots[0]] if len(slots) == 1 else
                         sum(res.g_scalar[k, s] for s in slots).to(torch.float32)).reshape(1, 1)
                elif kind == "row":
                    rows = self.d if slots[0] == _lib.P_THETA_Z else self.m
                    g = (gr32[k, slots[0], :rows] if len(slots) == 1 else
                         sum(res.g_row[k, s, :rows] for s in slots).to(torch.float32))
                    g = g.reshape(rows, 1)
                else:
                    g = (res.g_beta1 if kind == "elem1" else res.g_beta2)[k].to(torch.float32)
                    if cols is not None:
                        full = torch.zeros((self.m, self.batch_size), dtype=torch.float32,
                                           device=g.device)
                        full[:, cols[0]:cols[1]] = g
                        g = full
                out[key] = g
        if self._shared_weight():
            if any(rz[:nl]):
                out[self._fc_key(0)] = res.gW[0]
        else:
            for k in range(nl):
                if not rz[k]:
                    continue
                key = self._fc_key(k)
                out[key] = res.gW[k] if key not in out else out[key] + res.gW[k]
        return out

    def _shared_weight(self) -> bool:
        return isinstance(self.fc, nn.Linear)


def _shard_cols(t: torch.Tensor, batch: int, cols, name: str) -> torch.Tensor:
    c0, c1 = cols
    if t.dim() == 2 and t.shape[1] == batch and c1 - c0 != batch:
        return t[:, c0:c1].contiguous()
    if t.dim() == 2 and t.shape[1] == c1 - c0:
        return t
    raise ValueError(f"dladmm: {name} of shape {tuple(t.shape)} is neither the global batch "
                     f"({batch} columns) nor the shard's {c1 - c0}")


def _slice_tables(tables: dict, nl: int) -> dict:
    return {k: (v[:nl] if v is not None else None) for k, v in tables.items()}


def _train_precision(mod) -> str:
    if mod.precision not in ("f32", "f32_split"):
        raise RuntimeError(f"dladmm: precision {mod.precision!r} is inference-only "
                           "(training runs f32 or f32_split)")
    return mod.precision


class _DLADMMFunction(torch.autograd.Function):

    @staticmethod
    def forward(ctx, mod, x, nl, *params):
        dev = mod.A.device
        tables = _slice_tables(mod._tables(dev), nl)
        W = [w.detach() for w in mod._weights()[:nl]]
        r = dladmm_forward(mod.VARIANT, x, mod.A, W, mod.Z0, mod.E0, mod.L0, keep_all=True,
                           want_T=True, want_P=True, precision=_train_precision(mod),
                           p0_cache=mod._p0_cache(), **tables)
        ctx.mod = mod
        ctx.nl = nl
        ctx.tables = tables
        ctx.W = W
        ctx.fpath = r.path
        ctx.fflags = r.flags
        ctx.save_for_backward(x, r.Z, r.E, r.L, r.T, r.P)
        ctx.set_materialize_grads(False)
        K = nl
        outs = tuple(r.Z[k] for k in range(K)) + tuple(r.E[k] for k in range(K)) + \
            tuple(r.L[k] for k in range(K)) + tuple(r.T[j] for j in range(K + 1))
        if not mod.RETURNS_T:
            ctx.mark_non_differentiable(*outs[3 * K:])
        return outs

    @staticmethod
    def backward(ctx, *g):
        x, Z, E, L, T, P = ctx.saved_tensors
        mod = ctx.mod
        K = ctx.nl
        saved = ForwardResult(Z, E, L, T, None, P=P, path=ctx.fpath, flags=ctx.fflags)
        res = dladmm_backward(mod.VARIANT, x, mod.A, ctx.W, mod.Z0, mod.E0, mod.L0, saved,
                              g[:K], g[K:2 * K], g[2 * K:3 * K],
                              g[3 * K:] if mod.RETURNS_T else None,
                              tied=mod._shared_weight(), **ctx.tables)
        grads = mod._param_grads(res, K, _reachable(K, g, mod.RETURNS_T))
        names = [n for n, _ in mod.named_parameters()]
        return (None, None, None) + tuple(grads.get(n) for n in names)


_COEF: "OrderedDict" = OrderedDict()


def _coef_tensor(coeffs, dev) -> torch.Tensor:
    key = (str(dev), tuple(coeffs))
    c = _COEF.pop(key, None)
    if c is None:
        c = torch.as_tensor(list(coeffs), dtype=torch.float64, device=dev)
    _COEF[key] = c
    while len(_COEF) > 16:
        _COEF.popitem(last=False)
    return c


class _DLADMMLossFunction(torch.autograd.Function):

    @staticmethod
    def forward(ctx, mod, x, coeffs, alpha, kind, denom, cols, *params):
        dev = mod.A.device
        tables = mod._tables(dev, cols)
        W = [w.detach() for w in mod._weights()]
        Z0, E0, L0 = mod._init_state(cols)
        lk = {"l1l1": _lib.LOSS_L1L1, "lasso": _lib.LOSS_LASSO}[kind]
        r = dladmm_forward(mod.VARIANT, x, mod.A, W, Z0, E0, L0, keep_all=True, want_T=True,
                           loss_kind=lk, want_P=True, precision=_train_precision(mod),
                           p0_cache=mod._p0_cache(), **tables)
        per_layer = (alpha * r.loss_sums[:, 0] + r.loss_sums[:, 1]) / denom
        c = _coef_tensor(coeffs, dev)
        total = (c * per_layer).sum().to(torch.float32)
        ctx.mod, ctx.tables, ctx.W, ctx.lk, ctx.cols = mod, tables, W, lk, cols
        ctx.base = torch.stack([c * alpha / denom, c / denom], 1).to(torch.float32)
        ctx.fpath = r.path
        ctx.fflags = r.flags
        ctx.save_for_backward(x, r.Z, r.E, r.L, r.T, r.P)
        per_layer = per_layer.to(torch.float32)
        ctx.mark_non_differentiable(per_layer)
        return total, per_layer

    @staticmethod
    def backward(ctx, g_total, g_layers):
        x, Z, E, L, T, P = ctx.saved_tensors
        mod = ctx.mod
        K = mod.layers
        coef = (ctx.base * g_total).contiguous()
        Z0, E0, L0 = mod._init_state(ctx.cols)
        res = dladmm_backward(mod.VARIANT, x, mod.A, ctx.W, Z0, E0, L0,
                              ForwardResult(Z, E, L, T, None, P=P, path=ctx.fpath,
                                            flags=ctx.fflags),
                              loss_kind=ctx.lk,
                              loss_coef=coef,
                              tied=mod._shared_weight(), **ctx.tables)
        reach = {"z": [True] * K, "e": [k < K - 1 for k in range(K)],
                 "l": [k < K - 1 for k in range(K)]}
        grads = mod._param_grads(res, K, reach, ctx.cols)
        names = [n for n, _ in mod.named_parameters()]
        return (None,) * 7 + tuple(grads.get(n) for n in names)


class _DLADMMLenaLossFunction(torch.autograd.Function):

    @staticmethod
    def forward(ctx, mod, x, coeffs, alpha, denom, cols, lx_sign, save_cot, *params):
        dev = mod.A.device
        tables = mod._tables(dev, cols)
        W = [w.detach() for w in mod._weights()]
        Z0, E0, L0 = mod._init_state(cols)
        r = dladmm_forward(mod.VARIANT, x, mod.A, W, Z0, E0, L0, keep_all=True, want_T=True,
                           loss_kind=_lib.LOSS_L1L1, want_P=True, precision=_train_precision(mod),
                           p0_cache=mod._p0_cache(), **tables)
        c = _coef_tensor(coeffs, dev)
        c32 = c.to(torch.float32)
        ctx.grad = any(ctx.needs_input_grad[8:])
        if ctx.grad and save_cot:
            sums, gE, gL = dladmm_lena(x, mod.A, r.E, r.L, alpha, denom, coef=c32,
                                       lx_sign=lx_sign)
        else:
            sums = dladmm_lena(x, mod.A, r.E, r.L, alpha, denom, lx_sign=lx_sign)
            gE = gL = None
        per_layer = _lena_per_layer(r.loss_sums, sums, alpha, mod.A.shape, denom, lx_sign)
        total = (c * per_layer).sum().to(torch.float32)
        ctx.mod, ctx.tables, ctx.W, ctx.cols = mod, tables, W, cols
        ctx.alpha, ctx.denom, ctx.lx_sign = alpha, denom, lx_sign
        ctx.c = c32
        ctx.gEL = (gE, gL)
        ctx.fpath = r.path
        ctx.fflags = r.flags
        ctx.save_for_backward(x, r.Z, r.E, r.L, r.T, r.P)
        per_layer = per_layer.to(torch.float32)
        ctx.mark_non_differentiable(per_layer)
        return total, per_layer

    @staticmethod
    def backward(ctx, g_total, g_layers):
        x, Z, E, L, T, P = ctx.saved_tensors
        mod = ctx.mod
        K = mod.layers
        m, n = mod.A.shape
        ck = (ctx.c * g_total).contiguous()
        gE, gL = ctx.gEL if ctx.gEL is not None else (None, None)
        ctx.gEL = None
        if gE is None:
            gE, gL = dladmm_lena(x, mod.A, E, L, ctx.alpha, ctx.denom, coef=ctx.c, sums=False,
                                 lx_sign=ctx.lx_sign)
        g1 = g_total.to(torch.float32).reshape(1).contiguous()
        dladmm_scale_(gE, g1)
        dladmm_scale_(gL, g1)
        coef = torch.stack([ck * (ctx.alpha / (n * ctx.denom)), torch.zeros_like(ck)],
                           1).contiguous()
        Z0, E0, L0 = mod._init_state(ctx.cols)
        res = dladmm_backward(mod.VARIANT, x, mod.A, ctx.W, Z0, E0, L0,
                              ForwardResult(Z, E, L, T, None, P=P, path=ctx.fpath,
                                            flags=ctx.fflags),
                              gE=[gE[k] for k in range(K)], gL=[gL[k] for k in range(K)],
                              loss_kind=_lib.LOSS_L1L1, loss_coef=coef,
                              tied=mod._shared_weight(), **ctx.tables)
        reach = {"z": [True] * K, "e": [True] * K, "l": [True] * K}
        grads = mod._param_grads(res, K, reach, ctx.cols)
        names = [n_ for n_, _ in mod.named_parameters()]
        return (None,) * 8 + tuple(grads.get(n_) for n_ in names)


def _lena_per_layer(loss_sums, sums, alpha, shape, denom, lx_sign):
    m, n = shape
    return (alpha * loss_sums[:, 0] / n + sums[:, 1] / n +
            (sums[:, 0] + sums[:, 2] + lx_sign * sums[:, 3]) / m) / denom


def _reachable(K: int, g, has_t: bool) -> dict:
    def suffix(seq, n):
        out, acc = [False] * (n + 1), False
        for i in range(n - 1, -1, -1):
            acc = acc or (seq is not None and seq[i] is not None)
            out[i] = acc
        return out
    gZ, gE, gL = g[:K], g[K:2 * K], g[2 * K:3 * K]
    gT = g[3 * K:] if has_t else None
    sZ, sE, sL, sT = suffix(gZ, K), suffix(gE, K), suffix(gL, K), suffix(gT, K + 1)
    sT = sT + [False]
    re = [sE[k] or sL[k] or sT[k + 1] or sZ[k + 1] for k in range(K)]
    rl = [sL[k] or sZ[k + 1] or sE[k + 1] or sT[k + 2] for k in range(K)]
    rz = [sZ[k] or re[k] for k in range(K)]
    return {"z": rz, "e": re, "l": rl}


_SLOTS = {"b1": _lib.P_BETA1, "b2": _lib.P_BETA2, "b3": _lib.P_BETA3, "ss2": _lib.P_SS2,
          "ss2b": _lib.P_SS2B, "the": _lib.P_THETA_E, "thz": _lib.P_THETA_Z, "s1": _lib.P_S1}
_TABLE_IDX = {}


def _assemble_table(K: int, R: int, dev, spec: dict, rows: dict) -> torch.Tensor:
    tensors, layout = [], []
    consts = []
    for nm, src in spec.items():
        if isinstance(src, (int, float)):
            consts.append((nm, float(src)))
            continue
        seq = [src] * K if torch.is_tensor(src) else list(src)
        if len(seq) < K:
            raise ValueError(f"dladmm: {len(seq)} entries for parameter slot {nm}, need {K}")
        layout.append((nm, rows[nm]))
        tensors += [t.detach().reshape(-1) for t in seq[:K]]
    key = (str(dev), K, R, tuple(layout), tuple(consts))
    ent = _TABLE_IDX.get(key)
    if ent is None:
        idx = []
        for nm, nr in layout:
            for k in range(K):
                base = (k * _lib.NSCALAR + _SLOTS[nm]) * R
                idx.extend(range(base, base + nr))
        base_t = torch.zeros(K * _lib.NSCALAR * R, dtype=torch.float32)
        for nm, v in consts:
            for k in range(K):
                o = (k * _lib.NSCALAR + _SLOTS[nm]) * R
                base_t[o:o + R] = v
        ent = (torch.tensor(idx, dtype=torch.int64).to(dev), base_t.to(dev))
        _TABLE_IDX[key] = ent
    idx, base_t = ent
    out = base_t.clone()
    if tensors:
        flat = torch.cat(tensors).to(device=dev, dtype=torch.float32)
        if flat.numel() != idx.numel():
            raise ValueError("dladmm: parameter shapes do not match the table layout")
        out.index_copy_(0, idx, flat)
    return out.view(K, _lib.NSCALAR) if R == 1 else out.view(K, _lib.NSCALAR, R)


def _scalar_table(K, dev, **cols) -> torch.Tensor:
    t = torch.zeros((K, _lib.NSCALAR), dtype=torch.float32, device=dev)
    for k, v in cols.items():
        t[:, _SLOTS[k]] = v.to(device=dev, dtype=torch.float32) if torch.is_tensor(v) else v
    return t


class DLADMMNet(_DLADMMBase):
    VARIANT = _lib.V1_LENA
    GRAD_SLOTS = {"beta1": ("elem1", ()), "beta2": ("elem2", ())}
    PARAM_STEPS = dict(_DLADMMBase.PARAM_STEPS, beta1="zl")

    def _register_params(self):
        self.beta1 = nn.ParameterList()
        self.beta2 = nn.ParameterList()
        self.fc = nn.ModuleList()
        for _ in range(self.layers):
            self.beta1.append(nn.Parameter(torch.ones(self.m, self._pcols, dtype=torch.float32)))
            self.beta2.append(nn.Parameter(torch.ones(self.m, self._pcols, dtype=torch.float32)))
            self.fc.append(nn.Linear(self.m, self.d, bias=False))
        self.active_para = _dev(torch.tensor(0.025, dtype=torch.float32))
        self.active_para1 = _dev(torch.tensor(0.06, dtype=torch.float32))

    def _table_spec(self):
        return {"scalar": dict(thz=self.active_para.float(), the=self.active_para1.float(),
                               s1=1.0)}

    def _elem_param_lists(self) -> list:
        return [self.beta1, self.beta2]

    def _elem_betas(self, cols=None):
        def sl(b):
            b = b.detach()
            return b if cols is None else b[:, cols[0]:cols[1]].contiguous()
        return dict(beta1_elem=[sl(b) for b in self.beta1], beta2_elem=[sl(b) for b in self.beta2])


class DLADMMNetLTheta(_DLADMMBase):
    VARIANT = _lib.V2_LTHETA
    GRAD_SLOTS = {"beta1": ("row", (_lib.P_BETA1, _lib.P_BETA3)),
                  "beta2": ("row", (_lib.P_BETA2,)),
                  "active_para": ("row", (_lib.P_THETA_Z,)),
                  "active_para1": ("row", (_lib.P_THETA_E,))}
    PARAM_STEPS = dict(_DLADMMBase.PARAM_STEPS, beta1="zl")

    def _register_params(self):
        self._plist("beta1", (self.m, 1), 1.0)
        self._plist("beta2", (self.m, 1), 1.0)
        self._plist("active_para", (self.d, 1), 0.025)
        self._plist("active_para1", (self.m, 1), 0.06)
        self.fc = nn.ModuleList([nn.Linear(self.m, self.d, bias=False) for _ in range(self.layers)])

    def _table_spec(self):
        return {"row": dict(b1=self.beta1, b2=self.beta2, b3=self.beta1, the=self.active_para1,
                            thz=self.active_para)}


class DLADMMNetFull(_DLADMMBase):
    VARIANT = _lib.V3_FULL
    WSCALE = 0.4
    GRAD_SLOTS = {"beta1": ("row", (_lib.P_BETA1,)), "beta2": ("row", (_lib.P_BETA2,)),
                  "beta3": ("row", (_lib.P_BETA3,)), "ss2": ("row", (_lib.P_SS2,)),
                  "active_para": ("row", (_lib.P_THETA_Z,)),
                  "active_para1": ("row", (_lib.P_THETA_E,))}

    def _register_params(self):
        for nm in ("beta1", "beta2", "beta3", "ss2"):
            self._plist(nm, (self.m, 1), 1.0)
        self._plist("active_para", (self.d, 1), 0.2)
        self._plist("active_para1", (self.m, 1), 0.8)
        self.fc = nn.ModuleList([nn.Linear(self.m, self.d, bias=False) for _ in range(self.layers)])

    def _table_spec(self):
        return {"row": dict(b1=self.beta1, b2=self.beta2, b3=self.beta3, ss2=self.ss2,
                            the=self.active_para1, thz=self.active_para)}


class DLADMMNetScalar(_DLADMMBase):
    VARIANT = _lib.V4_SCALAR
    RETURNS_T = True
    WSCALE = 0.4
    NAME = "DLADMMNet_scalar"
    GRAD_SLOTS = {"beta1": ("scalar", (_lib.P_BETA1,)), "beta2": ("scalar", (_lib.P_BETA2,)),
                  "beta3": ("scalar", (_lib.P_BETA3,)), "ss2": ("scalar", (_lib.P_SS2,)),
                  "active_para": ("scalar", (_lib.P_THETA_Z,)),
                  "active_para1": ("scalar", (_lib.P_THETA_E,))}

    def __init__(self, m, n, d, batch_size, A, Z0, E0, L0, layers, **kw):
        super().__init__(m, n, d, batch_size, A, Z0, E0, L0, layers, **kw)
        self.At = self.A.t()
        A_np = A.detach().cpu().numpy()
        self.A_np = A_np
        self.L = _dev((np.linalg.norm(np.matmul(A_np.T, A_np), ord=2) * torch.ones(1, 1)).float())

    def _register_params(self):
        for nm in ("beta1", "beta2", "beta3", "ss2"):
            self._plist(nm, (1, 1), 1.0)
        self._plist("active_para", (1, 1), 0.2)
        self._plist("active_para1", (1, 1), 0.8)
        self.fc = nn.ModuleList([nn.Linear(self.m, self.d, bias=False) for _ in range(self.layers)])

    def _table_spec(self):
        return {"scalar": dict(b1=self.beta1, b2=self.beta2, b3=self.beta3, ss2=self.ss2,
                               the=self.active_para1, thz=self.active_para, s1=1.0)}


class DLADMMNetScalarSl2(DLADMMNetScalar):
    NAME = "DLADMMNet"


class DLADMMNetScalarZ0(DLADMMNetScalar):
    NAME = "DLADMMNet"


class DLADMMNetScalarTied(DLADMMNetScalar):
    VARIANT = _lib.V5_TIED
    NAME = "DLADMMNet_scalar_tied"
    GRAD_SLOTS = dict(DLADMMNetScalar.GRAD_SLOTS, ss1=("scalar", (_lib.P_S1,)))

    def _register_params(self):
        for nm in ("beta1", "beta2", "beta3", "ss1", "ss2"):
            self._plist(nm, (1, 1), 1.0)
        self._plist("active_para", (1, 1), 1e-4)
        self._plist("active_para1", (1, 1), 1e-2)
        self.fc = nn.Linear(self.m, self.d, bias=False)

    def _weights(self):
        return [self.fc.weight] * self.layers

    def _table_spec(self):
        return {"scalar": dict(b1=self.beta1, b2=self.beta2, b3=self.beta3, ss2=self.ss2,
                               the=self.active_para1, thz=self.active_para, s1=self.ss1)}


class DLADMMNetLasso(DLADMMNetScalar):
    VARIANT = _lib.V6_LASSO
    NAME = "DLADMMNet"
    GRAD_SLOTS = {"beta1": ("scalar", (_lib.P_BETA1,)), "beta3": ("scalar", (_lib.P_BETA3,)),
                  "ss2_1": ("scalar", (_lib.P_SS2,)), "ss2_2": ("scalar", (_lib.P_SS2B,)),
                  "active_para": ("scalar", (_lib.P_THETA_Z,))}

    def _register_params(self):
        self._plist("beta1", (1, 1), 1.0)
        self._plist("beta3", (1, 1), 1.0)
        self._plist("ss2_1", (1, 1), 0.5)
        self._plist("ss2_2", (1, 1), 0.5)
        self._plist("active_para", (1, 1), 0.2)
        self.fc = nn.ModuleList([nn.Linear(self.m, self.d, bias=False) for _ in range(self.layers)])

    def _table_spec(self):
        return {"scalar": dict(b1=self.beta1, b3=self.beta3, ss2=self.ss2_1, ss2b=self.ss2_2,
                               thz=self.active_para, s1=1.0)}


class DLADMMNetNewS(DLADMMNetScalar):
    NAME = "DLADMMNet_scalar_newS_layerwise"
    THZ0 = 0.1
    THE0 = 0.1

    def _register_params(self):
        for nm in ("beta1", "beta2", "beta3", "ss2"):
            self._plist(nm, (1, 1), 1.0)
        self._plist("active_para", (1, 1), self.THZ0)
        self._plist("active_para1", (1, 1), self.THE0)
        self.fc = nn.ModuleList([nn.Linear(self.m, self.d, bias=False) for _ in range(self.layers)])

    def forward(self, x, K=None):
        nl = self.layers if K is None else min(int(K), self.layers)
        Z, E, L, _T = self._forward_layers(x, nl)
        return Z, [self.E0] + E[: nl - 1], [self.L0] + L[: nl - 1]


class DLADMMNetTiedNewS(DLADMMNetNewS):
    VARIANT = _lib.V5_TIED
    NAME = "DLADMMNet_scalar_tied_newS_layerwise"
    THZ0 = 0.01
    THE0 = 0.01
    GRAD_SLOTS = dict(DLADMMNetScalar.GRAD_SLOTS, ss1=("scalar", (_lib.P_S1,)))

    def _register_params(self):
        for nm in ("beta1", "beta2", "beta3", "ss1", "ss2"):
            self._plist(nm, (1, 1), 1.0)
        self._plist("active_para", (1, 1), self.THZ0)
        self._plist("active_para1", (1, 1), self.THE0)
        self.fc = nn.Linear(self.m, self.d, bias=False)

    def _weights(self):
        return [self.fc.weight] * self.layers

    def _table_spec(self):
        return DLADMMNetScalarTied._table_spec(self)


class DLADMMNetPTiedNewS(DLADMMNetTiedNewS):
    NAME = "DLADMMNet_scalar_ptied_newS_layerwise"

    def __init__(self, m, n, d, batch_size, A, Z0, E0, L0, layers, interval, **kw):
        self.interval = interval
        super().__init__(m, n, d, batch_size, A, Z0, E0, L0, layers, **kw)

    def _register_params(self):
        for nm in ("beta1", "beta2", "beta3", "ss1", "ss2"):
            self._plist(nm, (1, 1), 1.0)
        self._plist("active_para", (1, 1), self.THZ0)
        self._plist("active_para1", (1, 1), self.THE0)
        self.fc = nn.ModuleList([nn.Linear(self.m, self.d, bias=False)
                                 for _ in range(self.layers // self.interval)])

    def _weights(self):
        return [self.fc[k // self.interval].weight for k in range(self.layers)]

    def _fc_key(self, k):
        return f"fc.{k // self.interval}.weight"

    def _shared_weight(self):
        return False

    def name(self):
        return "DLADMMNet_scalar_ptied{}_newS_layerwise".format(self.interval)


VARIANTS = {
    "v1": DLADMMNet, "v2": DLADMMNetLTheta, "v3": DLADMMNetFull,
    "v4": DLADMMNetScalar, "v4_sl2": DLADMMNetScalarSl2, "v4_z0": DLADMMNetScalarZ0,
    "v5": DLADMMNetScalarTied, "v6": DLADMMNetLasso,
    "v7": DLADMMNetNewS, "v7t": DLADMMNetTiedNewS, "v7p": DLADMMNetPTiedNewS,
}


def load_checkpoint(model: nn.Module, path: str, strict: bool = True):
    sd = torch.load(path, map_location="cpu", weights_only=True)
    if isinstance(sd, dict) and "state_dict" in sd and isinstance(sd["state_dict"], dict):
        sd = sd["state_dict"]
    return model.load_state_dict(sd, strict=strict)
```

### d-ladmm_amd/ops.py

```python
from __future__ import annotations

import contextlib
import contextvars
import ctypes
from dataclasses import dataclass
from typing import List, Optional, Sequence

import torch

from . import _lib


@dataclass
class ForwardResult:
    Z: torch.Tensor
    E: torch.Tensor
    L: torch.Tensor
    T: Optional[torch.Tensor]
    loss_sums: Optional[torch.Tensor]
    col_loss: Optional[torch.Tensor] = None
    P: Optional[torch.Tensor] = None
    path: int = 0
    flags: int = 0
    p0_reused: bool = False


_PLAN_FLAGS = contextvars.ContextVar("dladmm_plan_flags", default=0)
_FLAG_NAMES = {"per_layer": _lib.F_PER_LAYER, "bf16_wide": _lib.F_BF16_WIDE,
               "bwd_per_layer": _lib.F_BWD_PER_LAYER, "bwd_unfused": _lib.F_BWD_UNFUSED,
               "bwd_no_zmask": _lib.F_BWD_NO_ZMASK, "wgrad_f32": _lib.F_WGRAD_F32,
               "no_rowsplit": _lib.F_NO_ROWSPLIT, "no_xsplit": _lib.F_NO_XSPLIT,
               "rowsplit_rows": _lib.F_ROWSPLIT_ROWP}


@contextlib.contextmanager
def plan_flags(**opts):
    flags = _PLAN_FLAGS.get()
    for k, v in opts.items():
        if k not in _FLAG_NAMES:
            raise ValueError(f"dladmm: unknown plan flag {k!r} (one of {sorted(_FLAG_NAMES)})")
        flags = (flags | _FLAG_NAMES[k]) if v else (flags & ~_FLAG_NAMES[k])
    tok = _PLAN_FLAGS.set(flags)
    try:
        yield flags
    finally:
        _PLAN_FLAGS.reset(tok)


def _tensor_sig(t: torch.Tensor):
    try:
        return (t.data_ptr(), t._version, tuple(t.shape), tuple(t.stride()))
    except RuntimeError:
        return None


class PrologueCache:
    MAX_STREAMS = 4

    def __init__(self):
        from collections import OrderedDict
        self._slots = OrderedDict()

    def invalidate(self):
        self._slots.clear()

    def __deepcopy__(self, memo):
        return PrologueCache()

    def __reduce__(self):
        return (PrologueCache, ())

    def lookup(self, skey, key, nbytes, dev):
        slot = self._slots.pop(skey, None)
        hit = slot is not None and slot["key"] == key and slot["ws"].numel() >= nbytes
        if not hit:
            ws = slot["ws"] if slot is not None and slot["ws"].numel() >= nbytes else \
                torch.empty(max(nbytes, 1), device=dev, dtype=torch.uint8)
            slot = {"ws": ws, "key": None, "keep": None}
        self._slots[skey] = slot
        while len(self._slots) > self.MAX_STREAMS:
            self._slots.popitem(last=False)
        return slot["ws"], hit

    def commit(self, skey, key, keep):
        slot = self._slots.get(skey)
        if slot is not None:
            slot["key"], slot["keep"] = key, keep


def _f32_dev(t: torch.Tensor, name: str) -> torch.Tensor:
    if not isinstance(t, torch.Tensor):
        raise TypeError(f"dladmm: {name} must be a tensor")
    if t.device.type != "cuda":
        raise RuntimeError(f"dladmm: {name} is on {t.device}; the fused forward runs on a HIP "
                           "device only (no CPU fallback)")
    if t.dtype != torch.float32:
        raise TypeError(f"dladmm: {name} must be float32, got {t.dtype}")
    if t.dim() != 2 or (t.stride(1) != 1 and t.numel() > 0):
        raise ValueError(f"dladmm: {name} must be a 2-D row-major matrix (batch contiguous)")
    return t


def _fill_fwd_desc(d, variant, X, A, W, Z0, E0, L0, scalar_params, row_params, beta1_elem,
                   beta2_elem, keep_all, loss_kind, out, flags=None):
    X = _f32_dev(X, "X")
    A = _f32_dev(A, "A")
    Z0, E0, L0 = _f32_dev(Z0, "Z0"), _f32_dev(E0, "E0"), _f32_dev(L0, "L0")
    m, B = X.shape
    n = A.shape[1]
    K = len(W)
    if A.shape[0] != m:
        raise RuntimeError(f"dladmm: A is {tuple(A.shape)} but X has {m} rows")
    if tuple(Z0.shape) != (n, B) or tuple(E0.shape) != (m, B) or tuple(L0.shape) != (m, B):
        raise RuntimeError(
            "dladmm: Z0/E0/L0 shapes do not broadcast with X: "
            f"Z0 {tuple(Z0.shape)}, E0 {tuple(E0.shape)}, L0 {tuple(L0.shape)}, X {tuple(X.shape)}")
    if not 1 <= K <= _lib.MAX_LAYERS:
        raise ValueError(f"dladmm: layers must be in [1, {_lib.MAX_LAYERS}], got {K}")
    Ws = [_f32_dev(w if w.dim() == 2 and w.stride(1) == 1 else w.contiguous(), f"W[{k}]")
          for k, w in enumerate(W)]
    ldw = Ws[0].stride(0)
    for k, w in enumerate(Ws):
        if tuple(w.shape) != (n, m) or w.stride(0) != ldw:
            raise RuntimeError(f"dladmm: fc[{k}].weight must be ({n}, {m}) with a common stride")
    dev = X.device
    d.abi_version = _lib.ABI_VERSION
    d.flags = _PLAN_FLAGS.get() if flags is None else int(flags)
    d.variant, d.m, d.n, d.batch, d.layers = variant, m, n, B, K
    d.keep_all, d.loss_kind = int(bool(keep_all)), int(loss_kind)
    d.X, d.ld_x = X.data_ptr(), X.stride(0)
    d.A, d.ld_a = A.data_ptr(), A.stride(0)
    d.Z0, d.ld_z0 = Z0.data_ptr(), Z0.stride(0)
    d.E0, d.ld_e0 = E0.data_ptr(), E0.stride(0)
    d.L0, d.ld_l0 = L0.data_ptr(), L0.stride(0)
    warr = _lib.ptr_array([w.data_ptr() for w in Ws])
    d.W, d.ld_w = ctypes.cast(warr, ctypes.POINTER(ctypes.c_void_p)), ldw
    keep = [warr, Ws]
    if scalar_params is not None:
        sp = scalar_params
        if sp.device != dev or sp.dtype != torch.float32 or tuple(sp.shape) != (K, _lib.NSCALAR) \
                or not sp.is_contiguous():
            raise ValueError("dladmm: scalar_params must be a contiguous (K, 8) fp32 device tensor")
        d.scalar_params = sp.data_ptr()
    if row_params is not None:
        rp = row_params
        if rp.device != dev or rp.dtype != torch.float32 or rp.dim() != 3 or \
                rp.shape[0] != K or rp.shape[1] != _lib.NSCALAR or not rp.is_contiguous():
            raise ValueError("dladmm: row_params must be a contiguous (K, 8, R) fp32 device tensor")
        d.row_params, d.row_stride = rp.data_ptr(), rp.shape[2]
    if len(beta1_elem):
        b1 = [_f32_dev(b, f"beta1[{k}]") for k, b in enumerate(beta1_elem)]
        b2 = [_f32_dev(b, f"beta2[{k}]") for k, b in enumerate(beta2_elem)]
        ldb = b1[0].stride(0)
        for b in b1 + b2:
            if tuple(b.shape) != (m, B) or b.stride(0) != ldb:
                raise RuntimeError(
                    f"dladmm: per-sample beta of shape {tuple(b.shape)} does not broadcast with "
                    f"X {tuple(X.shape)} (main_lena.py:35-36 betas are (m, batch_size))")
        a1 = _lib.ptr_array([b.data_ptr() for b in b1])
        a2 = _lib.ptr_array([b.data_ptr() for b in b2])
        keep += [a1, a2]
        d.beta1_elem = ctypes.cast(a1, ctypes.POINTER(ctypes.c_void_p))
        d.beta2_elem = ctypes.cast(a2, ctypes.POINTER(ctypes.c_void_p))
        d.ld_beta = ldb
    d.Z, d.E, d.L = out.Z.data_ptr(), out.E.data_ptr(), out.L.data_ptr()
    d.T = out.T.data_ptr() if out.T is not None else None
    d.ld_out = B
    d.loss_sums = out.loss_sums.data_ptr() if out.loss_sums is not None else None
    d.P = out.P.data_ptr() if out.P is not None else None
    return keep


_PRECISIONS = {"f32": _lib.PREC_F32, "f32_split": _lib.PREC_F32_SPLIT, "bf16": _lib.PREC_BF16}


def dladmm_forward(variant: int, X: torch.Tensor, A: torch.Tensor, W: Sequence[torch.Tensor],
                   Z0: torch.Tensor, E0: torch.Tensor, L0: torch.Tensor, *,
                   scalar_params: Optional[torch.Tensor] = None,
                   row_params: Optional[torch.Tensor] = None,
                   beta1_elem: Sequence[torch.Tensor] = (),
                   beta2_elem: Sequence[torch.Tensor] = (),
                   keep_all: bool = True, want_T: bool = True, loss_kind: int = 0,
                   out: Optional[ForwardResult] = None,
                   kernel_events: Optional[tuple] = None,
                   want_col_loss: bool = False, precision: str = "f32",
                   want_P: bool = False, flags: Optional[int] = None,
                   p0_cache: Optional[PrologueCache] = None) -> ForwardResult:
    L = _lib.lib()
    _f32_dev(X, "X")
    _f32_dev(A, "A")
    m, B = X.shape
    n = A.shape[1]
    K = len(W)
    dev = X.device
    Kout = K if keep_all else 1
    if out is None:
        Zo = torch.empty((Kout, n, B), device=dev, dtype=torch.float32)
        Eo = torch.empty((Kout, m, B), device=dev, dtype=torch.float32)
        Lo = torch.empty((Kout, m, B), device=dev, dtype=torch.float32)
        To = (torch.empty((Kout + 1 if keep_all else 1, m, B), device=dev, dtype=torch.float32)
              if want_T else None)
        ls = torch.empty((K, 2), device=dev, dtype=torch.float64) if loss_kind else None
        out = ForwardResult(Zo, Eo, Lo, To, ls)
    out.flags = _PLAN_FLAGS.get() if flags is None else int(flags)

    if B == 0:
        _fill_fwd_desc(_lib.FwdDesc(), variant, X, A, W, Z0, E0, L0, scalar_params, row_params,
                       beta1_elem, beta2_elem, keep_all, loss_kind, out, out.flags)
        if out.loss_sums is not None:
            out.loss_sums.zero_()
        if want_col_loss:
            out.col_loss = torch.zeros((K, 2, 0), device=dev, dtype=torch.float32)
        if want_P and keep_all:
            out.P = torch.empty((K, m, 0), device=dev, dtype=torch.float32)
        return out
    d = _lib.FwdDesc()
    keep = _fill_fwd_desc(d, variant, X, A, W, Z0, E0, L0, scalar_params, row_params, beta1_elem,
                          beta2_elem, keep_all, loss_kind, out, out.flags)
    if precision not in _PRECISIONS:
        raise ValueError(f"dladmm: precision must be one of {sorted(_PRECISIONS)}, "
                         f"got {precision!r}")
    d.precision = _PRECISIONS[precision]
    if want_P and keep_all and out.P is None and L.dladmm_fwd_path(ctypes.byref(d)) in (1, 4, 5, 6):
        out.P = torch.empty((K, m, B), device=dev, dtype=torch.float32)
        d.P = out.P.data_ptr()
    if want_col_loss:
        if not loss_kind:
            raise ValueError("dladmm: per-column objectives need loss_kind")
        if out.col_loss is None:
            out.col_loss = torch.empty((K, 2, B), device=dev, dtype=torch.float32)
        d.col_loss = out.col_loss.data_ptr()
    if kernel_events is not None:
        d.ev_kernel_start = kernel_events[0].cuda_event
        d.ev_kernel_stop = kernel_events[1].cuda_event

    wsb = L.dladmm_fwd_workspace_bytes(ctypes.byref(d))
    if wsb == 0:
        path = L.dladmm_fwd_path(ctypes.byref(d))
        _lib.check(path if path < 0 else -7)
    out.path = L.dladmm_fwd_path(ctypes.byref(d))
    stream = torch.cuda.current_stream(dev).cuda_stream
    ws = ckey = None
    out.p0_reused = False
    if p0_cache is not None and out.path == 1 and not torch.cuda.is_current_stream_capturing():
        sa, sz = _tensor_sig(A), _tensor_sig(Z0)
        d.flags = out.flags | _lib.F_P0_SAVE
        wsb_p0 = L.dladmm_fwd_workspace_bytes(ctypes.byref(d))
        if sa is not None and sz is not None and wsb_p0 > wsb:
            ckey = (variant, m, n, B, K, precision, sa, sz, wsb_p0)
            skey = (dev.type, dev.index, stream)
            ws, out.p0_reused = p0_cache.lookup(skey, ckey, wsb_p0, dev)
            wsb = wsb_p0
            d.flags = (out.flags & ~_lib.F_P0_SAVE) | _lib.F_P0_REUSE if out.p0_reused \
                else out.flags | _lib.F_P0_SAVE
        else:
            d.flags = out.flags
    if ws is None:
        ws = _workspace(dev, wsb)
    d.workspace, d.workspace_bytes = ws.data_ptr(), wsb
    _lib.check(L.dladmm_fwd_f32(ctypes.byref(d), ctypes.c_void_p(stream)))
    if ckey is not None and not out.p0_reused:
        p0_cache.commit(skey, ckey, (A, Z0))
    del keep
    return out


@dataclass
class BackwardResult:
    gW: torch.Tensor
    g_scalar: Optional[torch.Tensor]
    g_row: Optional[torch.Tensor]
    g_beta1: List[torch.Tensor]
    g_beta2: List[torch.Tensor]
    path: int = 0


def dladmm_backward(variant: int, X: torch.Tensor, A: torch.Tensor, W: Sequence[torch.Tensor],
                    Z0: torch.Tensor, E0: torch.Tensor, L0: torch.Tensor, saved: ForwardResult,
                    gZ: Optional[Sequence] = None, gE: Optional[Sequence] = None,
                    gL: Optional[Sequence] = None, gT: Optional[Sequence] = None, *,
                    loss_kind: int = 0, loss_coef: Optional[torch.Tensor] = None,
                    scalar_params: Optional[torch.Tensor] = None,
                    row_params: Optional[torch.Tensor] = None,
                    beta1_elem: Sequence[torch.Tensor] = (),
                    beta2_elem: Sequence[torch.Tensor] = (),
                    tied: bool = False, flags: Optional[int] = None,
                    wgrad_split: Optional[bool] = None) -> BackwardResult:
    L = _lib.lib()
    if saved.T is None or saved.Z.shape[0] != len(W):
        raise ValueError("dladmm: backward needs the keep_all forward outputs including T")
    m, B = X.shape
    n = A.shape[1]
    K = len(W)
    dev = X.device
    if B == 0:
        gs = torch.zeros((K, _lib.NSCALAR), device=dev, dtype=torch.float64) \
            if variant >= _lib.V4_SCALAR else None
        gr = torch.zeros((K, _lib.NSCALAR, row_params.shape[2]), device=dev,
                         dtype=torch.float64) if variant in (_lib.V2_LTHETA, _lib.V3_FULL) else None
        gb = [torch.zeros((m, 0), device=dev) for _ in range(K)] if variant == _lib.V1_LENA \
            else []
        return BackwardResult(torch.zeros((1 if tied else K, n, m), device=dev), gs, gr, gb,
                              [t.clone() for t in gb])
    d = _lib.BwdDesc()
    if flags is None:
        flags = int(getattr(saved, "flags", 0)) | _PLAN_FLAGS.get()
    keep = _fill_fwd_desc(d.fwd, variant, X, A, W, Z0, E0, L0, scalar_params, row_params,
                          beta1_elem, beta2_elem, True, 0, saved, flags)
    split = saved.path == 4 if wgrad_split is None else bool(wgrad_split)
    d.fwd.precision = _PRECISIONS["f32_split"] if split else _PRECISIONS["f32"]
    counts = {"gZ": (K, n), "gE": (K, m), "gL": (K, m), "gT": (K + 1, m)}
    for nm, seq in (("gZ", gZ), ("gE", gE), ("gL", gL), ("gT", gT)):
        if seq is None or all(g is None for g in seq):
            continue
        cnt, rows = counts[nm]
        if len(seq) != cnt:
            raise ValueError(f"dladmm: {nm} must have {cnt} entries")
        ptrs = []
        for g in seq:
            if g is None:
                ptrs.append(None)
                continue
            if tuple(g.shape) != (rows, B) or g.dtype != torch.float32 or g.device != dev:
                raise ValueError(f"dladmm: {nm} entries must be fp32 ({rows}, {B}) device tensors")
            g = g.contiguous()
            keep.append(g)
            ptrs.append(g.data_ptr())
        arr = _lib.ptr_array(ptrs)
        keep.append(arr)
        setattr(d, nm, ctypes.cast(arr, ctypes.POINTER(ctypes.c_void_p)))
    d.ld_g = B
    if loss_kind:
        if loss_coef is None or tuple(loss_coef.shape) != (K, 2) or loss_coef.dtype != \
                torch.float32 or loss_coef.device != dev or not loss_coef.is_contiguous():
            raise ValueError("dladmm: loss_coef must be a contiguous fp32 (K, 2) device tensor")
        d.loss_kind, d.loss_coef = int(loss_kind), loss_coef.data_ptr()
    gWo = torch.empty((1 if tied else K, n, m), device=dev, dtype=torch.float32)
    d.gW, d.ld_gw = gWo.data_ptr(), m
    d.gw_sum = int(bool(tied))
    g_scalar = g_row = None
    g1, g2 = [], []
    if variant >= _lib.V4_SCALAR:
        g_scalar = torch.zeros((K, _lib.NSCALAR), device=dev, dtype=torch.float64)
        d.g_scalar = g_scalar.data_ptr()
    elif variant in (_lib.V2_LTHETA, _lib.V3_FULL):
        g_row = torch.zeros((K, _lib.NSCALAR, d.fwd.row_stride), device=dev, dtype=torch.float64)
        d.g_row = g_row.data_ptr()
    else:
        g1 = [torch.empty((m, B), device=dev, dtype=torch.float32) for _ in range(K)]
        g2 = [torch.empty((m, B), device=dev, dtype=torch.float32) for _ in range(K)]
        if d.fwd.ld_beta != B:
            raise ValueError("dladmm: V1 backward needs contiguous (m, B) betas")
        a1 = _lib.ptr_array([t.data_ptr() for t in g1])
        a2 = _lib.ptr_array([t.data_ptr() for t in g2])
        keep += [a1, a2]
        d.g_beta1_elem = ctypes.cast(a1, ctypes.POINTER(ctypes.c_void_p))
        d.g_beta2_elem = ctypes.cast(a2, ctypes.POINTER(ctypes.c_void_p))
    wsb = L.dladmm_bwd_workspace_bytes(ctypes.byref(d))
    if wsb == 0:
        raise ValueError("dladmm: invalid backward descriptor")
    path = L.dladmm_bwd_path(ctypes.byref(d))
    ws = _workspace(dev, wsb)
    d.workspace, d.workspace_bytes = ws.data_ptr(), wsb
    stream = torch.cuda.current_stream(dev).cuda_stream
    _lib.check(L.dladmm_bwd_f32(ctypes.byref(d), ctypes.c_void_p(stream)))
    del keep
    return BackwardResult(gWo, g_scalar, g_row, g1, g2, path)


def dladmm_scale_(x: torch.Tensor, s: torch.Tensor) -> torch.Tensor:
    if x.dtype != torch.float32 or not x.is_contiguous() or s.dtype != torch.float32 or \
            s.numel() != 1 or s.device != x.device or x.device.type != "cuda":
        raise ValueError("dladmm: scale needs a contiguous fp32 tensor and an fp32 device scalar")
    s = s.contiguous()
    stream = torch.cuda.current_stream(x.device).cuda_stream
    _lib.check(_lib.lib().dladmm_scale_f32(ctypes.c_void_p(x.data_ptr()), x.numel(),
                                           ctypes.c_void_p(s.data_ptr()), ctypes.c_void_p(stream)))
    return x


def dladmm_lena(X: torch.Tensor, A: torch.Tensor, E: torch.Tensor, L: torch.Tensor, alpha: float,
                denom: float, coef: Optional[torch.Tensor] = None, sums: bool = True,
                lx_sign: float = 1.0):
    Lb = _lib.lib()
    if lx_sign not in (1.0, -1.0):
        raise ValueError(f"dladmm: lx_sign must be +1 or -1 (got {lx_sign})")
    K, m, B = L.shape
    n = A.shape[1]
    dev = X.device
    for t in (E, L):
        if tuple(t.shape) != (K, m, B) or t.dtype != torch.float32 or not t.is_contiguous():
            raise ValueError("dladmm: E and L must be contiguous fp32 (K, m, B) tensors")
    if tuple(X.shape) != (m, B) or tuple(A.shape) != (m, n) or X.dtype != torch.float32 or \
            A.dtype != torch.float32:
        raise ValueError(f"dladmm: X must be fp32 ({m}, {B}) and A fp32 ({m}, n); got "
                         f"{tuple(X.shape)} {X.dtype}, {tuple(A.shape)} {A.dtype}")
    if dev.type != "cuda" or any(t.device != dev for t in (A, E, L)):
        raise ValueError("dladmm: X, A, E and L must be on one GPU")
    if K == 0 or B == 0:
        sm = torch.zeros((K, 4), device=dev, dtype=torch.float64)
        gE, gL = torch.zeros_like(E), torch.zeros_like(L)
        if coef is None:
            return sm
        return (sm, gE, gL) if sums else (gE, gL)
    X = X.contiguous()
    A = A.contiguous()
    d = _lib.LenaDesc()
    d.abi_version = _lib.ABI_VERSION
    d.m, d.n, d.batch, d.layers = m, n, B, K
    d.alpha = float(alpha)
    d.lx_negate = 1 if lx_sign < 0 else 0
    d.inv_mb, d.inv_nb = 1.0 / (m * float(denom)), 1.0 / (n * float(denom))
    d.X, d.ld_x = X.data_ptr(), X.stride(0)
    d.A, d.ld_a = A.data_ptr(), A.stride(0)
    d.E, d.L, d.layer_stride, d.ld = E.data_ptr(), L.data_ptr(), m * B, B
    sm = gE = gL = None
    if coef is None or sums:
        sm = torch.empty((K, 4), device=dev, dtype=torch.float64)
        d.sums = sm.data_ptr()
    if coef is not None:
        if tuple(coef.shape) != (K,) or coef.dtype != torch.float32 or coef.device != dev:
            raise ValueError("dladmm: coef must be an fp32 (K,) device tensor")
        coef = coef.contiguous()
        gE = torch.empty((K, m, B), device=dev, dtype=torch.float32)
        gL = torch.empty((K, m, B), device=dev, dtype=torch.float32)
        d.gE, d.gL, d.g_layer_stride, d.ld_g = gE.data_ptr(), gL.data_ptr(), m * B, B
        d.coef = coef.data_ptr()
    d.mode = 0 if coef is None else (2 if sums else 1)
    out = sm if coef is None else ((sm, gE, gL) if sums else (gE, gL))
    wsb = Lb.dladmm_lena_workspace_bytes(ctypes.byref(d))
    if wsb == 0:
        raise ValueError(f"dladmm: the fused main_lena objective supports m <= 256, n <= 512 "
                         f"(got m={m}, n={n}, K={K}, B={B})")
    ws = _workspace(dev, wsb)
    d.workspace, d.workspace_bytes = ws.data_ptr(), wsb
    stream = torch.cuda.current_stream(dev).cuda_stream
    _lib.check(Lb.dladmm_lena_f32(ctypes.byref(d), ctypes.c_void_p(stream)))
    return out


_WS: "OrderedDict" = None
_WS_PER_DEVICE = 4


def _workspace(dev: torch.device, nbytes: int) -> torch.Tensor:
    global _WS
    from collections import OrderedDict
    if _WS is None:
        _WS = OrderedDict()
    stream = torch.cuda.current_stream(dev)
    key = (dev.type, dev.index, stream.cuda_stream)
    buf = _WS.pop(key, None)
    if buf is None or buf.numel() < nbytes:
        buf = torch.empty(max(nbytes, 1), device=dev, dtype=torch.uint8)
    _WS[key] = buf
    same = [k for k in _WS if k[:2] == key[:2]]
    for k in same[:-_WS_PER_DEVICE]:
        del _WS[k]
    return buf
```

### include/dladmm.h

```cpp
#ifndef DLADMM_H_
#define DLADMM_H_

#include <stddef.h>
#include <stdint.h>

#ifdef __cplusplus
extern "C" {
#endif

#define DLADMM_ABI_VERSION 6
#define DLADMM_MAX_LAYERS 65536

enum dladmm_variant {
  DLADMM_V1_LENA = 1,
  DLADMM_V2_LTHETA = 2,
  DLADMM_V3_FULL = 3,
  DLADMM_V4_SCALAR = 4,
  DLADMM_V5_TIED = 5,
  DLADMM_V6_LASSO = 6,
  DLADMM_V7_SCALAR_V1E = 7
};

enum dladmm_loss_kind {
  DLADMM_LOSS_NONE = 0,
  DLADMM_LOSS_L1L1 = 1,
  DLADMM_LOSS_LASSO = 2
};

#define DLADMM_E_ABI_VERSION (-1)
#define DLADMM_E_VARIANT (-2)
#define DLADMM_E_SHAPE (-3)
#define DLADMM_E_LAYERS (-4)
#define DLADMM_E_NULL (-5)
#define DLADMM_E_WORKSPACE (-6)
#define DLADMM_E_UNSUPPORTED (-7)
#define DLADMM_E_ALIGN (-8)

enum dladmm_param_slot {
  DLADMM_P_BETA1 = 0,
  DLADMM_P_BETA2 = 1,
  DLADMM_P_BETA3 = 2,
  DLADMM_P_SS2 = 3,
  DLADMM_P_SS2B = 4,
  DLADMM_P_THETA_E = 5,
  DLADMM_P_THETA_Z = 6,
  DLADMM_P_S1 = 7,
  DLADMM_NSCALAR = 8
};

typedef struct dladmm_fwd_desc {
  int32_t abi_version;
  int32_t variant;
  int32_t m;
  int32_t n;
  int32_t batch;
  int32_t layers;
  int32_t keep_all;
  int32_t loss_kind;

  const float* X;  int64_t ld_x;
  const float* A;  int64_t ld_a;
  const float* Z0; int64_t ld_z0;
  const float* E0; int64_t ld_e0;
  const float* L0; int64_t ld_l0;

  const float* const* W; int64_t ld_w;

  const float* scalar_params;
  const float* row_params; int64_t row_stride;
  const float* const* beta1_elem;
  const float* const* beta2_elem;
  int64_t ld_beta;

  float* Z; float* E; float* L; float* T;
  int64_t ld_out;

  double* loss_sums;

  void* workspace; size_t workspace_bytes;

  void* ev_kernel_start;
  void* ev_kernel_stop;

  float* col_loss;

  int32_t precision;
  int32_t flags;

  float* P;
} dladmm_fwd_desc;

enum dladmm_precision { DLADMM_PREC_F32 = 0, DLADMM_PREC_BF16 = 1, DLADMM_PREC_F32_SPLIT = 2 };

enum dladmm_flags {
  DLADMM_F_PER_LAYER = 1,
  DLADMM_F_BF16_WIDE = 2,
  DLADMM_F_BWD_PER_LAYER = 4,
  DLADMM_F_BWD_UNFUSED = 8,
  DLADMM_F_BWD_NO_ZMASK = 16,
  DLADMM_F_WGRAD_F32 = 32,
  DLADMM_F_NO_ROWSPLIT = 64,
  DLADMM_F_NO_XSPLIT = 128,
  DLADMM_F_ROWSPLIT_ROWP = 256,
  DLADMM_F_P0_SAVE = 512,
  DLADMM_F_P0_REUSE = 1024,
  DLADMM_F_ELZ = 2048,
  DLADMM_F_ELZ_TAIL = 4096
};

int dladmm_abi_version(void);

size_t dladmm_fwd_workspace_bytes(const dladmm_fwd_desc* d);

int dladmm_fwd_path(const dladmm_fwd_desc* d);

int dladmm_fwd_f32(const dladmm_fwd_desc* d, void* stream);

typedef struct dladmm_bwd_desc {
  dladmm_fwd_desc fwd;

  const float* const* gZ;
  const float* const* gE;
  const float* const* gL;
  const float* const* gT;
  int64_t ld_g;

  int32_t loss_kind;
  int32_t gw_sum;
  const float* loss_coef;

  float* gW; int64_t ld_gw;
  double* g_scalar;
  double* g_row;
  float* const* g_beta1_elem;
  float* const* g_beta2_elem;

  void* workspace; size_t workspace_bytes;
} dladmm_bwd_desc;

size_t dladmm_bwd_workspace_bytes(const dladmm_bwd_desc* d);

int dladmm_bwd_path(const dladmm_bwd_desc* d);

int dladmm_bwd_f32(const dladmm_bwd_desc* d, void* stream);

enum dladmm_mu_updater {
  DLADMM_MU_NONE = 0,
  DLADMM_MU_EMA = 1,
  DLADMM_MU_GS = 2,
  DLADMM_MU_RT = 3
};

typedef struct dladmm_safeguard_desc {
  int32_t abi_version;
  int32_t m, n, batch;
  int64_t ld;
  const float *Zl, *El, *Ll, *Tl;
  const float *Zk, *Ek, *Lk, *Tk;
  const float *Es, *Ts;
  const float* Ep;
  float *Zo, *Eo, *Lo, *To;
  float* mu;
  float* norm_out;
  int32_t* count;
  float beta, c;
  double delta;
  int32_t updater;
  float mu_param;
} dladmm_safeguard_desc;

int dladmm_safeguard_f32(const dladmm_safeguard_desc* d, void* stream);

typedef struct dladmm_safeguard_news_desc {
  int32_t abi_version;
  int32_t m, n, batch;
  int64_t ld;
  const float* X;
  const float *Zl, *El, *Ll;
  const float *Zk, *Ek, *Lk;
  const float *En, *Znn;
  const float *Pn, *Pnn;
  float *Zo, *Eo, *Lo;
  float* mu;
  float* norm_out;
  int32_t* count;
  uint8_t* mask;
  const float* inv_bs;
  double delta;
  int32_t updater;
  float mu_param;
} dladmm_safeguard_news_desc;

int dladmm_safeguard_news_f32(const dladmm_safeguard_news_desc* d, void* stream);

typedef struct dladmm_colobj_desc {
  int32_t abi_version;
  int32_t m, n, batch, layers;
  int32_t fit_kind;
  const float* Z; int64_t z_layer_stride; int64_t ld_z;
  const float* E; int64_t e_layer_stride; int64_t ld_e;
  const float* T; int64_t t_layer_stride; int64_t ld_t;
  const float* Zref; int64_t ld_zref;
  const float* Eref; int64_t ld_eref;
  double* reg; double* fit; double* dz; double* de;
} dladmm_colobj_desc;

int dladmm_colobj_f32(const dladmm_colobj_desc* d, void* stream);

typedef struct dladmm_lena_desc {
  int32_t abi_version;
  int32_t m, n, batch, layers;
  int32_t mode;
  float alpha, inv_mb, inv_nb;
  int32_t lx_negate;
  const float* X; int64_t ld_x;
  const float* A; int64_t ld_a;
  const float* E; const float* L; int64_t layer_stride; int64_t ld;
  double* sums;
  float* gE; float* gL; int64_t g_layer_stride; int64_t ld_g;
  const float* coef;
  void* workspace; size_t workspace_bytes;
} dladmm_lena_desc;

size_t dladmm_lena_workspace_bytes(const dladmm_lena_desc* d);
int dladmm_lena_f32(const dladmm_lena_desc* d, void* stream);

int dladmm_scale_f32(float* x, int64_t n, const float* s, void* stream);

const char* dladmm_error_string(int code);

#ifdef __cplusplus
}
#endif
#endif
```

Baseline: 15.77 million samples/s.

## Assemble per-layer parameter table on device, fused into the weight-pack launch

Instead of building the (K,8,R) scalar/row parameter table in PyTorch with many small ops before each forward, the model now passes raw parameter tensor pointers. A new prep kernel gathers them into a workspace table, and that work is folded into the existing W-pack launch. This targets host-side op dispatch and the small-kernel launches that precede the main fused kernel. In exchange it adds a new C API, ctypes struct building per call, extra workspace, and changes to the P0 cache key.

```diff
diff --git a/d-ladmm_amd/_lib.py b/d-ladmm_amd/_lib.py
--- a/d-ladmm_amd/_lib.py
+++ b/d-ladmm_amd/_lib.py
@@ -26,7 +26,8 @@
 P_BETA1, P_BETA2, P_BETA3, P_SS2, P_SS2B, P_THETA_E, P_THETA_Z, P_S1 = range(8)
 
 EXPORTED = ("dladmm_abi_version", "dladmm_fwd_workspace_bytes", "dladmm_fwd_path",
-            "dladmm_fwd_f32", "dladmm_bwd_workspace_bytes", "dladmm_bwd_path", "dladmm_bwd_f32",
+            "dladmm_fwd_f32", "dladmm_fwd_workspace_bytes_src", "dladmm_fwd_path_src",
+            "dladmm_fwd_f32_src", "dladmm_bwd_workspace_bytes", "dladmm_bwd_path", "dladmm_bwd_f32",
             "dladmm_safeguard_f32", "dladmm_safeguard_news_f32", "dladmm_colobj_f32", "dladmm_lena_workspace_bytes",
             "dladmm_lena_f32", "dladmm_scale_f32", "dladmm_error_string")
 MU_NONE, MU_EMA, MU_GS, MU_RT = 0, 1, 2, 3
@@ -62,6 +63,20 @@
     ]
 
 
+PREP_SRCS = 112
+EVERY_LAYER = -1
+
+
+class ParamSrc(ctypes.Structure):
+    _fields_ = [("ptr", _fp), ("slot", _i32), ("layer", _i32), ("count", _i32),
+                ("reserved", _i32)]
+
+
+class ParamSrcs(ctypes.Structure):
+    _fields_ = [("src", ctypes.POINTER(ParamSrc)), ("nsrc", _i32), ("reserved", _i32),
+                ("slot_const", ctypes.c_float * NSCALAR)]
+
+
 class BwdDesc(ctypes.Structure):
     _fields_ = [
         ("fwd", FwdDesc),
@@ -149,6 +164,13 @@
     L.dladmm_fwd_path.argtypes = [ctypes.POINTER(FwdDesc)]
     L.dladmm_fwd_f32.restype = ctypes.c_int
     L.dladmm_fwd_f32.argtypes = [ctypes.POINTER(FwdDesc), ctypes.c_void_p]
+    L.dladmm_fwd_workspace_bytes_src.restype = ctypes.c_size_t
+    L.dladmm_fwd_workspace_bytes_src.argtypes = [ctypes.POINTER(FwdDesc), ctypes.POINTER(ParamSrcs)]
+    L.dladmm_fwd_path_src.restype = ctypes.c_int
+    L.dladmm_fwd_path_src.argtypes = [ctypes.POINTER(FwdDesc), ctypes.POINTER(ParamSrcs)]
+    L.dladmm_fwd_f32_src.restype = ctypes.c_int
+    L.dladmm_fwd_f32_src.argtypes = [ctypes.POINTER(FwdDesc), ctypes.POINTER(ParamSrcs),
+                                     ctypes.c_void_p]
     L.dladmm_bwd_workspace_bytes.restype = ctypes.c_size_t
     L.dladmm_bwd_workspace_bytes.argtypes = [ctypes.POINTER(BwdDesc)]
     L.dladmm_bwd_path.restype = ctypes.c_int
diff --git a/d-ladmm_amd/csrc/dladmm_capi.hip b/d-ladmm_amd/csrc/dladmm_capi.hip
--- a/d-ladmm_amd/csrc/dladmm_capi.hip
+++ b/d-ladmm_amd/csrc/dladmm_capi.hip
@@ -26,7 +26,7 @@
 };
 static_assert(sizeof(PackArgs) <= 2048, "kernel argument size");
 
-__global__ __launch_bounds__(256) void pack_frags_kernel(const PackArgs p) {
+__device__ __forceinline__ void pack_frags_body(const PackArgs& p) {
   const int t = blockIdx.y;
   const int64_t fr = (int64_t)blockIdx.x * 4 + (threadIdx.x >> 6);
   if (fr >= (int64_t)p.RB * p.CB) return;
@@ -80,6 +80,57 @@
                : 0.0f;
   reinterpret_cast<f32x4*>(p.dst)[((int64_t)t * p.RB * p.CB + fr) * 64 + lane] = v;
 }
+__global__ __launch_bounds__(256) void pack_frags_kernel(const PackArgs p) { pack_frags_body(p); }
+
+constexpr int kPrepSrcs = DLADMM_PREP_SRCS;
+struct PrepEnt {
+  const float* p;
+  int where;
+  int count;
+};
+struct PrepArgs {
+  PackArgs pk;
+  int nb;
+  int n, nall;
+  int K, R;
+  int fill;
+  unsigned named;
+  float* dst;
+  float cst[DLADMM_NSCALAR];
+  PrepEnt e[kPrepSrcs];
+};
+static_assert(sizeof(PrepArgs) <= 3072, "kernel argument size");
+static_assert(kPrepSrcs >= 7 * 15, "K = 15 with seven per-layer slots (V5) fits one launch");
+
+__global__ __launch_bounds__(256) void prep_kernel(const PrepArgs a) {
+  if ((int)blockIdx.y < a.nb) {
+    pack_frags_body(a.pk);
+    return;
+  }
+  const int64_t tid = (int64_t)blockIdx.x * 256 + threadIdx.x;
+  const int64_t nth = (int64_t)gridDim.x * 256;
+  const int R = a.R;
+  const int64_t per = (int64_t)(a.n - a.nall) * R;
+  for (int64_t i = tid; i < per; i += nth) {
+    const PrepEnt& s = a.e[a.nall + (int)(i / R)];
+    const int r = (int)(i % R);
+    a.dst[(int64_t)s.where * R + r] = r < s.count ? s.p[r] : 0.0f;
+  }
+  const int64_t kr = (int64_t)a.K * R;
+  for (int j = 0; j < a.nall; ++j) {
+    const PrepEnt& s = a.e[j];
+    const int slot = -s.where - 1;
+    for (int64_t i = tid; i < kr; i += nth) {
+      const int r = (int)(i % R);
+      a.dst[((i / R) * DLADMM_NSCALAR + slot) * R + r] = r < s.count ? s.p[r] : 0.0f;
+    }
+  }
+  if (a.fill)
+    for (int64_t i = tid; i < kr * DLADMM_NSCALAR; i += nth) {
+      const int slot = (int)((i / R) % DLADMM_NSCALAR);
+      if (!((a.named >> slot) & 1u)) a.dst[i] = a.cst[slot];
+    }
+}
 
 __global__ __launch_bounds__(256) void zero_fill_kernel(uint32_t* p, int64_t words,
                                                         uint8_t* tail, int ntail) {
@@ -299,11 +350,14 @@
   bool p0;
   size_t off_p0;
   int64_t ldzw;
+  bool ptab;
+  size_t off_ptab;
+  int ptab_rows;
 };
 
 inline bool fits_32bit(const dladmm_fwd_desc* d);
 
-inline int validate(const dladmm_fwd_desc* d) {
+inline int validate(const dladmm_fwd_desc* d, bool have_src = false) {
   if (!d) return DLADMM_E_NULL;
   if (d->abi_version != DLADMM_ABI_VERSION) return DLADMM_E_ABI_VERSION;
   if (d->variant < DLADMM_V1_LENA || d->variant > DLADMM_V7_SCALAR_V1E) return DLADMM_E_VARIANT;
@@ -321,9 +375,9 @@
     return DLADMM_E_UNSUPPORTED;
   const int v = d->variant;
   if (v == DLADMM_V2_LTHETA || v == DLADMM_V3_FULL) {
-    if (!d->row_params) return DLADMM_E_NULL;
+    if (!d->row_params && !have_src) return DLADMM_E_NULL;
     if (d->row_stride < d->m || d->row_stride < d->n) return DLADMM_E_SHAPE;
-  } else if (!d->scalar_params) {
+  } else if (!d->scalar_params && !have_src) {
     return DLADMM_E_NULL;
   }
   if (v == DLADMM_V1_LENA) {
@@ -493,9 +547,114 @@
   return 0;
 }
 
+inline bool have_srcs(const dladmm_param_srcs* ps) { return ps && ps->nsrc != 0; }
+
+inline int validate_srcs(const dladmm_fwd_desc* d, const dladmm_param_srcs* ps) {
+  if (ps->nsrc < 0) return DLADMM_E_SHAPE;
+  if (!ps->src) return DLADMM_E_NULL;
+  const bool rows = d->variant == DLADMM_V2_LTHETA || d->variant == DLADMM_V3_FULL;
+  const int64_t R = rows ? d->row_stride : 1;
+  const int K = d->layers;
+  if ((int64_t)K * DLADMM_NSCALAR * R >= ((int64_t)1 << 31)) return DLADMM_E_UNSUPPORTED;
+  int all[DLADMM_NSCALAR] = {}, per[DLADMM_NSCALAR] = {};
+  std::vector<bool> seen;
+  for (int i = 0; i < ps->nsrc; ++i) {
+    const dladmm_param_src& s = ps->src[i];
+    if (!s.ptr) return DLADMM_E_NULL;
+    if (s.slot < 0 || s.slot >= DLADMM_NSCALAR || s.count < 1 || s.count > R)
+      return DLADMM_E_SHAPE;
+    if (s.layer == DLADMM_EVERY_LAYER) {
+      ++all[s.slot];
+    } else {
+      if (s.layer < 0 || s.layer >= K) return DLADMM_E_SHAPE;
+      if (seen.empty()) seen.assign((size_t)K * DLADMM_NSCALAR, false);
+      const size_t w = (size_t)s.layer * DLADMM_NSCALAR + s.slot;
+      if (seen[w]) return DLADMM_E_SHAPE;
+      seen[w] = true;
+      ++per[s.slot];
+    }
+  }
+  for (int sl = 0; sl < DLADMM_NSCALAR; ++sl)
+    if (all[sl] > 1 || (all[sl] && per[sl]) || (per[sl] && per[sl] != K)) return DLADMM_E_SHAPE;
+  return 0;
+}
+
+inline int plan_with_srcs(const dladmm_fwd_desc* d, const dladmm_param_srcs* ps, Plan* p) {
+  const bool src = have_srcs(ps);
+  if (int e = validate(d, src)) return e;
+  if (src)
+    if (int e = validate_srcs(d, ps)) return e;
+  if (int e = make_plan(d, p)) return e;
+  if (src) {
+    const bool rows = d->variant == DLADMM_V2_LTHETA || d->variant == DLADMM_V3_FULL;
+    p->ptab = true;
+    p->ptab_rows = rows ? (int)d->row_stride : 1;
+    p->off_ptab = p->total;
+    p->total += align256((size_t)d->layers * DLADMM_NSCALAR * p->ptab_rows * sizeof(float));
+  }
+  return 0;
+}
+
+struct PrepJob {
+  const dladmm_param_srcs* ps;
+  float* dst;
+  int K, R;
+};
+
 inline hipError_t pack(const float* const* srcs, int T, int R, int C, int64_t ld, int RB, int CB,
                        int order, float* dst, hipStream_t s, float sign = 1.0f,
-                       const float* scal = nullptr, int trans = 0, int t0 = 0, int bf16 = 0) {
+                       const float* scal = nullptr, int trans = 0, int t0 = 0, int bf16 = 0,
+                       const PrepJob* job = nullptr) {
+  if (job) {
+    const dladmm_param_srcs& ps = *job->ps;
+    std::vector<const dladmm_param_src*> ord;
+    ord.reserve(ps.nsrc);
+    unsigned named = 0;
+    for (int pass = 0; pass < 2; ++pass)
+      for (int i = 0; i < ps.nsrc; ++i)
+        if ((ps.src[i].layer == DLADMM_EVERY_LAYER) == (pass == 0)) ord.push_back(&ps.src[i]);
+    for (int i = 0; i < ps.nsrc; ++i) named |= 1u << ps.src[i].slot;
+    const int nl_pack = (T + kPackBatch - 1) / kPackBatch;
+    const int nl_tab = (ps.nsrc + kPrepSrcs - 1) / kPrepSrcs;
+    const int nl = nl_pack > nl_tab ? nl_pack : nl_tab;
+    for (int l = 0; l < nl; ++l) {
+      PrepArgs a{};
+      const int b = l * kPackBatch;
+      const int nb = b >= T ? 0 : (T - b < kPackBatch ? T - b : kPackBatch);
+      PackArgs& pa = a.pk;
+      pa.trans = trans; pa.t0 = t0 + b;
+      for (int t = 0; t < nb; ++t) pa.src[t] = srcs[b + t];
+      pa.R = R; pa.C = C; pa.RB = RB; pa.CB = CB; pa.order = order; pa.ld = ld;
+      pa.dst = dst + (size_t)b * RB * CB * kFrag;
+      pa.sign = sign; pa.scal = scal; pa.bf16 = bf16;
+      pa.vec = ld % 4 == 0 ? 1 : 0;
+      for (int t = 0; t < nb; ++t)
+        if ((uintptr_t)pa.src[t] & 15) pa.vec = 0;
+      a.nb = nb;
+      const int e0 = l * kPrepSrcs;
+      a.n = e0 >= ps.nsrc ? 0 : (ps.nsrc - e0 < kPrepSrcs ? ps.nsrc - e0 : kPrepSrcs);
+      for (int i = 0; i < a.n; ++i) {
+        const dladmm_param_src& q = *ord[e0 + i];
+        const bool every = q.layer == DLADMM_EVERY_LAYER;
+        a.e[i].p = q.ptr;
+        a.e[i].where = every ? -(q.slot + 1) : q.layer * DLADMM_NSCALAR + q.slot;
+        a.e[i].count = q.count;
+        if (every) a.nall = i + 1;
+      }
+      a.K = job->K; a.R = job->R; a.dst = job->dst;
+      a.fill = l == 0 ? 1 : 0;
+      a.named = named;
+      for (int sl = 0; sl < DLADMM_NSCALAR; ++sl) a.cst[sl] = ps.slot_const[sl];
+      int gx = (RB * CB + 3) / 4;
+      if (nb == 0) {
+        const int64_t work = (int64_t)job->K * DLADMM_NSCALAR * job->R;
+        gx = (int)((work + 255) / 256 < 64 ? (work + 255) / 256 : 64);
+      }
+      hipLaunchKernelGGL(prep_kernel, dim3(gx < 1 ? 1 : gx, nb + 1), dim3(256), 0, s, a);
+      if (hipError_t e = hipGetLastError()) return e;
+    }
+    return hipSuccess;
+  }
   for (int b = 0; b < T; b += kPackBatch) {
     const int nb = T - b < kPackBatch ? T - b : kPackBatch;
     PackArgs pa{};
@@ -525,7 +684,8 @@
 #endif
 }
 
-inline int run_fused(const dladmm_fwd_desc* d, const Plan& p, char* ws, hipStream_t s) {
+inline int run_fused(const dladmm_fwd_desc* d, const Plan& p, char* ws, hipStream_t s,
+                     const PrepJob* job = nullptr) {
   float* Ap = (float*)(ws + p.off_ap);
   float* Wp = (float*)(ws + p.off_wp);
   float* lossp = (float*)(ws + p.off_loss);
@@ -536,7 +696,7 @@
   if (!p0_reuse)
     if (hipError_t e = pack(asrc, 1, d->m, d->n, d->ld_a, MB, NB, 2, Ap, s)) return (int)e;
   if (hipError_t e = pack(d->W, shared ? 1 : d->layers, d->n, d->m, d->ld_w, NB, MB, 2, Wp, s,
-                          -1.0f))
+                          -1.0f, nullptr, 0, 0, 0, job))
     return (int)e;
   FusedArgs a{};
   a.m = d->m; a.n = d->n; a.B = d->batch; a.K = d->layers;
@@ -581,7 +741,8 @@
     a.xch = (float*)(ws + p.off_xch);
     a.xstride = (int64_t)xs_group_floats();
     a.xcnt = (unsigned*)(ws + p.off_xcnt);
-    if (hipError_t e = zero_async(a.xcnt, p.total - p.off_xcnt, s)) return (int)e;
+    if (hipError_t e = zero_async(a.xcnt, (p.ptab ? p.off_ptab : p.total) - p.off_xcnt, s))
+      return (int)e;
   }
   hipError_t e = p.path == 6 ? launch_fused_xs(p.shape, d->variant, a, s)
                  : p.path == 5
@@ -1359,31 +1520,51 @@
 int dladmm_abi_version(void) { return DLADMM_ABI_VERSION; }
 
 size_t dladmm_fwd_workspace_bytes(const dladmm_fwd_desc* d) {
+  return dladmm_fwd_workspace_bytes_src(d, nullptr);
+}
+
+size_t dladmm_fwd_workspace_bytes_src(const dladmm_fwd_desc* d, const dladmm_param_srcs* ps) {
   using namespace dladmm;
-  if (validate(d)) return 0;
   Plan p;
-  if (make_plan(d, &p)) return 0;
-  return p.total;
-}
-
-int dladmm_fwd_path(const dladmm_fwd_desc* d) {
+  return plan_with_srcs(d, ps, &p) ? 0 : p.total;
+}
+
+int dladmm_fwd_path(const dladmm_fwd_desc* d) { return dladmm_fwd_path_src(d, nullptr); }
+
+int dladmm_fwd_path_src(const dladmm_fwd_desc* d, const dladmm_param_srcs* ps) {
   using namespace dladmm;
-  if (int e = validate(d)) return e;
   Plan p;
-  if (int e = make_plan(d, &p)) return e;
+  if (int e = plan_with_srcs(d, ps, &p)) return e;
   return p.path;
 }
 
 int dladmm_fwd_f32(const dladmm_fwd_desc* d, void* stream) {
+  return dladmm_fwd_f32_src(d, nullptr, stream);
+}
+
+int dladmm_fwd_f32_src(const dladmm_fwd_desc* d0, const dladmm_param_srcs* ps, void* stream) {
   using namespace dladmm;
-  if (int e = validate(d)) return e;
   Plan p;
-  if (int e = make_plan(d, &p)) return e;
-  if (!d->workspace || d->workspace_bytes < p.total) return DLADMM_E_WORKSPACE;
-  if (((uintptr_t)d->workspace) & 255) return DLADMM_E_ALIGN;
+  if (int e = plan_with_srcs(d0, ps, &p)) return e;
+  if (!d0->workspace || d0->workspace_bytes < p.total) return DLADMM_E_WORKSPACE;
+  if (((uintptr_t)d0->workspace) & 255) return DLADMM_E_ALIGN;
   hipStream_t s = (hipStream_t)stream;
-  char* ws = (char*)d->workspace;
-  const int rc = p.path == 1 || p.path >= 5 ? run_fused(d, p, ws, s)
+  char* ws = (char*)d0->workspace;
+  dladmm_fwd_desc dsrc;
+  const dladmm_fwd_desc* d = d0;
+  PrepJob job{};
+  if (p.ptab) {
+    job.ps = ps; job.dst = (float*)(ws + p.off_ptab); job.K = d0->layers; job.R = p.ptab_rows;
+    dsrc = *d0;
+    if (d0->variant == DLADMM_V2_LTHETA || d0->variant == DLADMM_V3_FULL) dsrc.row_params = job.dst;
+    else dsrc.scalar_params = job.dst;
+    d = &dsrc;
+    if (!(p.path == 1 || p.path >= 5))
+      if (hipError_t e = pack(nullptr, 0, 0, 0, 0, 0, 0, 0, nullptr, s, 1.0f, nullptr, 0, 0, 0,
+                              &job))
+        return (int)e;
+  }
+  const int rc = p.path == 1 || p.path >= 5 ? run_fused(d, p, ws, s, p.ptab ? &job : nullptr)
                  : p.path == 4 ? run_fused_x3(d, p, ws, s)
                                : run_layered(d, p, ws, s);
   if (rc) return rc;
diff --git a/d-ladmm_amd/model.py b/d-ladmm_amd/model.py
--- a/d-ladmm_amd/model.py
+++ b/d-ladmm_amd/model.py
@@ -8,8 +8,8 @@
 import torch.nn as nn
 
 from . import _lib
-from .ops import (ForwardResult, PrologueCache, dladmm_backward, dladmm_forward, dladmm_lena,
-                  dladmm_scale_)
+from .ops import (ForwardResult, ParamSources, PrologueCache, dladmm_backward, dladmm_forward,
+                  dladmm_lena, dladmm_scale_)
 
 
 def _dev(t: torch.Tensor) -> torch.Tensor:
@@ -118,13 +118,18 @@
     def _elem_betas(self, cols=None) -> dict:
         return {}
 
-    def _tables(self, dev, cols=None) -> dict:
+    native_tables = True
+
+    def _tables(self, dev, cols=None, native=False) -> dict:
         out = {}
         for kind, spec in self._table_spec().items():
             R = 1 if kind == "scalar" else max(self.m, self.d)
             rows = {nm: (1 if kind == "scalar" else (self.d if nm == "thz" else self.m))
                     for nm in spec}
-            out[f"{kind}_params"] = _assemble_table(self.layers, R, dev, spec, rows)
+            if native and self.native_tables:
+                out["param_srcs"] = _param_sources(self.layers, R, spec, rows)
+            else:
+                out[f"{kind}_params"] = _assemble_table(self.layers, R, dev, spec, rows)
         out.update(self._elem_betas(cols))
         return out
 
@@ -156,7 +161,8 @@
                 self.VARIANT, x, self.A, [w.detach() for w in self._weights()],
                 self.Z0, self.E0, self.L0, keep_all=keep_all, want_T=self.RETURNS_T,
                 loss_kind=loss_kind, kernel_events=kernel_events, want_col_loss=want_col_loss,
-                precision=self.precision, p0_cache=self._p0_cache(), **self._tables(dev))
+                precision=self.precision, p0_cache=self._p0_cache(),
+                **self._tables(dev, native=True))
 
     def _forward_layers(self, x, nl: int):
         if self._needs_grad():
@@ -170,7 +176,7 @@
             return (list(outs[:nl]), list(outs[nl:2 * nl]), list(outs[2 * nl:3 * nl]),
                     list(outs[3 * nl:]))
         with torch.no_grad():
-            tables = _slice_tables(self._tables(self.A.device), nl)
+            tables = _slice_tables(self._tables(self.A.device, native=True), nl)
             r = dladmm_forward(self.VARIANT, x, self.A, [w.detach() for w in self._weights()[:nl]],
                                self.Z0, self.E0, self.L0, keep_all=True, want_T=self.RETURNS_T,
                                precision=self.precision, p0_cache=self._p0_cache(), **tables)
@@ -254,7 +260,7 @@
         kw.setdefault("precision", self.precision)
         kw.setdefault("p0_cache", self._p0_cache())
         return dladmm_forward(self.VARIANT, x, self.A, W, Z0, E0, L0, keep_all=True,
-                              **kw, **self._tables(dev, cols))
+                              **kw, **self._tables(dev, cols, native=True))
 
     GRAD_SLOTS: dict = {}
     PARAM_STEPS = {"beta1": "z", "beta2": "e", "beta3": "l", "ss2": "e", "ss2_1": "e",
@@ -317,7 +323,8 @@
 
 
 def _slice_tables(tables: dict, nl: int) -> dict:
-    return {k: (v[:nl] if v is not None else None) for k, v in tables.items()}
+    return {k: (None if v is None else v.first(nl) if isinstance(v, ParamSources) else v[:nl])
+            for k, v in tables.items()}
 
 
 def _train_precision(mod) -> str:
@@ -553,6 +560,21 @@
     return out.view(K, _lib.NSCALAR) if R == 1 else out.view(K, _lib.NSCALAR, R)
 
 
+def _param_sources(K: int, R: int, spec: dict, rows: dict) -> ParamSources:
+    tensors, layout, consts = [], [], [0.0] * _lib.NSCALAR
+    for nm, src in spec.items():
+        if isinstance(src, (int, float)):
+            consts[_SLOTS[nm]] = float(src)
+            continue
+        every = torch.is_tensor(src)
+        seq = [src] if every else list(src)[:K]
+        if len(seq) < (1 if every else K):
+            raise ValueError(f"dladmm: {len(seq)} entries for parameter slot {nm}, need {K}")
+        layout.append((_SLOTS[nm], every, rows[nm]))
+        tensors += seq
+    return ParamSources(R, K, layout, tensors, consts)
+
+
 def _scalar_table(K, dev, **cols) -> torch.Tensor:
     t = torch.zeros((K, _lib.NSCALAR), dtype=torch.float32, device=dev)
     for k, v in cols.items():
diff --git a/d-ladmm_amd/ops.py b/d-ladmm_amd/ops.py
--- a/d-ladmm_amd/ops.py
+++ b/d-ladmm_amd/ops.py
@@ -6,6 +6,7 @@
 from dataclasses import dataclass
 from typing import List, Optional, Sequence
 
+import numpy as np
 import torch
 
 from . import _lib
@@ -88,6 +89,60 @@
             slot["key"], slot["keep"] = key, keep
 
 
+class ParamSources:
+    __slots__ = ("rows", "layers", "layout", "tensors", "consts")
+
+    def __init__(self, rows, layers, layout, tensors, consts):
+        self.rows, self.layers, self.layout = int(rows), int(layers), tuple(layout)
+        self.tensors, self.consts = list(tensors), tuple(float(c) for c in consts)
+
+    def first(self, nl: int) -> "ParamSources":
+        if nl == self.layers:
+            return self
+        ts, i = [], 0
+        for _slot, every, _cnt in self.layout:
+            ts += self.tensors[i:i + (1 if every else nl)]
+            i += 1 if every else self.layers
+        return ParamSources(self.rows, nl, self.layout, ts, self.consts)
+
+
+_SRC_TMPL = {}
+
+
+def _param_srcs_struct(ps: ParamSources, K: int, dev):
+    if ps.layers != K:
+        raise ValueError(f"dladmm: parameter sources of {ps.layers} layers for a {K}-layer call")
+    key = (K, ps.layout)
+    tmpl = _SRC_TMPL.get(key)
+    if tmpl is None:
+        words = []
+        for slot, every, cnt in ps.layout:
+            for k in ([_lib.EVERY_LAYER] if every else range(K)):
+                words.append((0, (slot & 0xFFFFFFFF) | ((k & 0xFFFFFFFF) << 32), cnt))
+        tmpl = np.array(words, dtype=np.uint64).reshape(-1, 3)
+        cnts = [int(c) for c in tmpl[:, 2]]
+        tmpl = _SRC_TMPL[key] = (tmpl, cnts)
+    tmpl, cnts = tmpl
+    ts = ps.tensors
+    if len(ts) != len(cnts):
+        raise ValueError("dladmm: parameter shapes do not match the table layout")
+    keep = []
+    for i, t in enumerate(ts):
+        if t.dtype is not torch.float32 or t.device != dev or not t.is_contiguous():
+            ts = list(ts) if ts is ps.tensors else ts
+            ts[i] = t = t.detach().to(device=dev, dtype=torch.float32).contiguous()
+        if t.numel() != cnts[i]:
+            raise ValueError("dladmm: parameter shapes do not match the table layout")
+    arr = tmpl.copy()
+    arr[:, 0] = [t.data_ptr() for t in ts]
+    s = _lib.ParamSrcs()
+    s.src = ctypes.cast(arr.ctypes.data, ctypes.POINTER(_lib.ParamSrc))
+    s.nsrc = len(ts)
+    s.slot_const[:] = ps.consts
+    keep += [arr, ts]
+    return s, keep
+
+
 def _f32_dev(t: torch.Tensor, name: str) -> torch.Tensor:
     if not isinstance(t, torch.Tensor):
         raise TypeError(f"dladmm: {name} must be a tensor")
@@ -102,7 +157,7 @@
 
 
 def _fill_fwd_desc(d, variant, X, A, W, Z0, E0, L0, scalar_params, row_params, beta1_elem,
-                   beta2_elem, keep_all, loss_kind, out, flags=None):
+                   beta2_elem, keep_all, loss_kind, out, flags=None, param_srcs=None):
     X = _f32_dev(X, "X")
     A = _f32_dev(A, "A")
     Z0, E0, L0 = _f32_dev(Z0, "Z0"), _f32_dev(E0, "E0"), _f32_dev(L0, "L0")
@@ -148,6 +203,10 @@
                 rp.shape[0] != K or rp.shape[1] != _lib.NSCALAR or not rp.is_contiguous():
             raise ValueError("dladmm: row_params must be a contiguous (K, 8, R) fp32 device tensor")
         d.row_params, d.row_stride = rp.data_ptr(), rp.shape[2]
+    if param_srcs is not None:
+        if scalar_params is not None or row_params is not None:
+            raise ValueError("dladmm: pass a parameter table or parameter sources, not both")
+        d.row_stride = param_srcs.rows
     if len(beta1_elem):
         b1 = [_f32_dev(b, f"beta1[{k}]") for k, b in enumerate(beta1_elem)]
         b2 = [_f32_dev(b, f"beta2[{k}]") for k, b in enumerate(beta2_elem)]
@@ -185,7 +244,8 @@
                    kernel_events: Optional[tuple] = None,
                    want_col_loss: bool = False, precision: str = "f32",
                    want_P: bool = False, flags: Optional[int] = None,
-                   p0_cache: Optional[PrologueCache] = None) -> ForwardResult:
+                   p0_cache: Optional[PrologueCache] = None,
+                   param_srcs: Optional[ParamSources] = None) -> ForwardResult:
     L = _lib.lib()
     _f32_dev(X, "X")
     _f32_dev(A, "A")
@@ -206,7 +266,7 @@
 
     if B == 0:
         _fill_fwd_desc(_lib.FwdDesc(), variant, X, A, W, Z0, E0, L0, scalar_params, row_params,
-                       beta1_elem, beta2_elem, keep_all, loss_kind, out, out.flags)
+                       beta1_elem, beta2_elem, keep_all, loss_kind, out, out.flags, param_srcs)
         if out.loss_sums is not None:
             out.loss_sums.zero_()
         if want_col_loss:
@@ -216,12 +276,18 @@
         return out
     d = _lib.FwdDesc()
     keep = _fill_fwd_desc(d, variant, X, A, W, Z0, E0, L0, scalar_params, row_params, beta1_elem,
-                          beta2_elem, keep_all, loss_kind, out, out.flags)
+                          beta2_elem, keep_all, loss_kind, out, out.flags, param_srcs)
+    ps = None
+    if param_srcs is not None:
+        srcs, skeep = _param_srcs_struct(param_srcs, K, dev)
+        keep += skeep
+        ps = ctypes.byref(srcs)
     if precision not in _PRECISIONS:
         raise ValueError(f"dladmm: precision must be one of {sorted(_PRECISIONS)}, "
                          f"got {precision!r}")
     d.precision = _PRECISIONS[precision]
-    if want_P and keep_all and out.P is None and L.dladmm_fwd_path(ctypes.byref(d)) in (1, 4, 5, 6):
+    if want_P and keep_all and out.P is None and \
+            L.dladmm_fwd_path_src(ctypes.byref(d), ps) in (1, 4, 5, 6):
         out.P = torch.empty((K, m, B), device=dev, dtype=torch.float32)
         d.P = out.P.data_ptr()
     if want_col_loss:
@@ -234,23 +300,26 @@
         d.ev_kernel_start = kernel_events[0].cuda_event
         d.ev_kernel_stop = kernel_events[1].cuda_event
 
-    wsb = L.dladmm_fwd_workspace_bytes(ctypes.byref(d))
+    wsb = L.dladmm_fwd_workspace_bytes_src(ctypes.byref(d), ps)
     if wsb == 0:
-        path = L.dladmm_fwd_path(ctypes.byref(d))
+        path = L.dladmm_fwd_path_src(ctypes.byref(d), ps)
         _lib.check(path if path < 0 else -7)
-    out.path = L.dladmm_fwd_path(ctypes.byref(d))
+    out.path = L.dladmm_fwd_path_src(ctypes.byref(d), ps)
     stream = torch.cuda.current_stream(dev).cuda_stream
     ws = ckey = None
     out.p0_reused = False
     if p0_cache is not None and out.path == 1 and not torch.cuda.is_current_stream_capturing():
         sa, sz = _tensor_sig(A), _tensor_sig(Z0)
         d.flags = out.flags | _lib.F_P0_SAVE
-        wsb_p0 = L.dladmm_fwd_workspace_bytes(ctypes.byref(d))
+        wsb_p0 = L.dladmm_fwd_workspace_bytes_src(ctypes.byref(d), ps)
         if sa is not None and sz is not None and wsb_p0 > wsb:
-            ckey = (variant, m, n, B, K, precision, sa, sz, wsb_p0)
+            R = d.row_stride if variant in (_lib.V2_LTHETA, _lib.V3_FULL) else 1
+            tab = (K * _lib.NSCALAR * R * 4 + 255) // 256 * 256
+            lay = wsb_p0 - tab if ps is not None else wsb_p0
+            ckey = (variant, m, n, B, K, precision, sa, sz, lay)
             skey = (dev.type, dev.index, stream)
-            ws, out.p0_reused = p0_cache.lookup(skey, ckey, wsb_p0, dev)
-            wsb = wsb_p0
+            ws, out.p0_reused = p0_cache.lookup(skey, ckey, lay + tab, dev)
+            wsb = lay + tab
             d.flags = (out.flags & ~_lib.F_P0_SAVE) | _lib.F_P0_REUSE if out.p0_reused \
                 else out.flags | _lib.F_P0_SAVE
         else:
@@ -258,7 +327,7 @@
     if ws is None:
         ws = _workspace(dev, wsb)
     d.workspace, d.workspace_bytes = ws.data_ptr(), wsb
-    _lib.check(L.dladmm_fwd_f32(ctypes.byref(d), ctypes.c_void_p(stream)))
+    _lib.check(L.dladmm_fwd_f32_src(ctypes.byref(d), ps, ctypes.c_void_p(stream)))
     if ckey is not None and not out.p0_reused:
         p0_cache.commit(skey, ckey, (A, Z0))
     del keep
diff --git a/include/dladmm.h b/include/dladmm.h
--- a/include/dladmm.h
+++ b/include/dladmm.h
@@ -115,6 +115,28 @@
 int dladmm_fwd_path(const dladmm_fwd_desc* d);
 
 int dladmm_fwd_f32(const dladmm_fwd_desc* d, void* stream);
+
+#define DLADMM_PREP_SRCS 112
+#define DLADMM_EVERY_LAYER (-1)
+
+typedef struct dladmm_param_src {
+  const float* ptr;
+  int32_t slot;
+  int32_t layer;
+  int32_t count;
+  int32_t reserved;
+} dladmm_param_src;
+
+typedef struct dladmm_param_srcs {
+  const dladmm_param_src* src;
+  int32_t nsrc;
+  int32_t reserved;
+  float slot_const[DLADMM_NSCALAR];
+} dladmm_param_srcs;
+
+size_t dladmm_fwd_workspace_bytes_src(const dladmm_fwd_desc* d, const dladmm_param_srcs* ps);
+int dladmm_fwd_path_src(const dladmm_fwd_desc* d, const dladmm_param_srcs* ps);
+int dladmm_fwd_f32_src(const dladmm_fwd_desc* d, const dladmm_param_srcs* ps, void* stream);
 
 typedef struct dladmm_bwd_desc {
   dladmm_fwd_desc fwd;
```

Measured after the change: 15.79 million samples/s (median of 5 runs). No clear change (+0.1%).
